# Zydak/Vulkan-Path-Tracer

Measured on AMD Instinct MI355X. Metric: Msamples/s at 1920x1080, higher is better.
Workload: dtype f32; 1 GPU; cornell_1080p_d8; scene=CornellBox (12 triangles, emissive quad 50), black env, width=1920, height=1080, max_depth=8, samples_per_frame=1, batches_per_gpu=14 x 904 frames, partition=rows y % N == rank, one ncclGather at the end, base_seed=1

## Files before the change

### include/vpt_lab.h

```cpp
#ifndef VPT_LAB_H
#define VPT_LAB_H
#include "vpt.h"
#ifdef __cplusplus
extern "C" {
#endif

#define VPT_TRACE_BASE 0u
#define VPT_TRACE_VOTE 1u
#define VPT_TRACE_VOTE8 2u
#define VPT_TRACE_POOL 3u
#define VPT_TRACE_PAIR 4u
#define VPT_TRACE_VOTE4S 5u
int vpt_lab_set_rays(vpt_ctx* ctx, const vpt_ray* rays_host, uint32_t n);
#define VPT_LAB_LANES 1u
#define VPT_LAB_LANE_GRID 2u
#define VPT_LAB_TAIL_GRID 3u
#define VPT_LAB_WHOLE_FRAMES 4u
#define VPT_LAB_WHOLE_SCHED 5u
#define VPT_LAB_WHOLE_PARTS 6u
#define VPT_LAB_WHOLE_CULL 7u
int vpt_lab_set(vpt_ctx* ctx, uint32_t key, uint32_t value);
int vpt_lab_whole_culled(const vpt_ctx* ctx, uint64_t* out);
int vpt_lab_trace(vpt_ctx* ctx, uint32_t variant, uint32_t any_hit, const uint32_t* order_host, uint32_t param, uint32_t reps,
                  vpt_hit* hits_host, float* best_ms, uint64_t* visits);
int vpt_lab_set_holes(vpt_ctx* ctx, const unsigned char* hole_host);
int vpt_lab_trace_shadow(vpt_ctx* ctx, uint32_t light, uint32_t ray_queries, const uint32_t* expect_host, const unsigned char* media_host,
                         const unsigned char* hole_host, unsigned char* vis_host, uint64_t* visits);

#ifdef __cplusplus
}
#endif
#endif
```

### vulkan-path-tracer_amd/_abi.py

```python
import ctypes as C

VPT_OK = 0
ERR_NAMES = {
    -1: "VPT_ERR_INVALID_ARGUMENT", -2: "VPT_ERR_NO_DEVICE", -3: "VPT_ERR_OUT_OF_MEMORY", -4: "VPT_ERR_NO_SCENE",
    -5: "VPT_ERR_DEVICE", -6: "VPT_ERR_UNSUPPORTED", -7: "VPT_ERR_LIMIT",
}

FLAG_SKY_MIS = 1 << 0
FLAG_MESH_MIS = 1 << 1
FLAG_LOCAL_HITS = 1 << 8
FLAG_SHOW_ENV_DIRECTLY = 1 << 2
FLAG_GEOMETRY_NORMALS = 1 << 3
FLAG_ENERGY_COMPENSATION = 1 << 4
FLAG_FURNACE = 1 << 5
FLAG_RAY_QUERIES = 1 << 6
FLAG_TONEMAP_LINEAR_BLOOM_TAP = 1 << 7
FLAGS_DEFAULT = (FLAG_SKY_MIS | FLAG_MESH_MIS | FLAG_SHOW_ENV_DIRECTLY | FLAG_ENERGY_COMPENSATION |
                 FLAG_RAY_QUERIES | FLAG_TONEMAP_LINEAR_BLOOM_TAP)

KERNEL_NAMES = ["primary", "extend", "shade", "connect", "bounce", "resolve", "bloom", "tonemap", "shadow", "join"]
KERNEL_COUNT = 10
PIPELINE_AUTO, PIPELINE_FUSED, PIPELINE_STAGED = 0, 1, 2
PIPELINE_STAGED_R1, PIPELINE_STAGED_SORTED, PIPELINE_WHOLE = 3, 4, 5
LAB_LANES, LAB_LANE_GRID, LAB_TAIL_GRID, LAB_WHOLE_FRAMES, LAB_WHOLE_SCHED, LAB_WHOLE_PARTS, LAB_WHOLE_CULL = 1, 2, 3, 4, 5, 6, 7
ASYNC_MAX_BOUNCES = 32


class Material(C.Structure):
    _fields_ = [
        ("base_color", C.c_float * 3), ("emissive_color", C.c_float * 3), ("specular_color", C.c_float * 3),
        ("medium_color", C.c_float * 3), ("medium_emissive_color", C.c_float * 3),
        ("metallic", C.c_float), ("roughness", C.c_float), ("ior", C.c_float), ("transmission", C.c_float),
        ("anisotropy", C.c_float), ("anisotropy_rotation", C.c_float), ("medium_density", C.c_float),
        ("medium_anisotropy", C.c_float),
        ("base_color_texture", C.c_uint32), ("normal_texture", C.c_uint32), ("roughness_texture", C.c_uint32),
        ("metallic_texture", C.c_uint32), ("emissive_texture", C.c_uint32),
    ]


assert C.sizeof(Material) == 112


class Volume(C.Structure):
    _fields_ = [
        ("corner_min", C.c_float * 3), ("corner_max", C.c_float * 3), ("color", C.c_float * 3), ("emissive_color", C.c_float * 3),
        ("density", C.c_float), ("anisotropy", C.c_float), ("alpha", C.c_float), ("droplet_size", C.c_float),
        ("density_data_index", C.c_int32), ("approximated_scattering", C.c_int32), ("approximated_scattering_falloff", C.c_float),
        ("grid_sharpness", C.c_float), ("has_temperature_data", C.c_int32), ("use_blackbody", C.c_int32), ("temperature_color", C.c_float * 3),
        ("temperature_gamma", C.c_float), ("temperature_scale", C.c_float), ("emissive_color_gamma", C.c_float),
        ("kelvin_min", C.c_int32), ("kelvin_max", C.c_int32),
    ]


assert C.sizeof(Volume) == 120


class Atmosphere(C.Structure):
    _fields_ = [
        ("planet_position", C.c_float * 3), ("planet_radius", C.c_float), ("atmosphere_height", C.c_float),
        ("rayleigh_density_falloff", C.c_float), ("mie_density_falloff", C.c_float), ("ozone_density_falloff", C.c_float),
        ("ozone_peak", C.c_float),
        ("rayleigh_multiplier", C.c_float * 3), ("mie_multiplier", C.c_float * 3), ("ozone_multiplier", C.c_float * 3),
        ("sun_color", C.c_float * 3),
    ]


assert C.sizeof(Atmosphere) == 84


def atmosphere(**kw):
    a = Atmosphere()
    d = dict(planet_position=(0.0, 6360e3 + 1000.0, 0.0), planet_radius=6360e3, atmosphere_height=100e3, rayleigh_density_falloff=8000.0,
             mie_density_falloff=1200.0, ozone_density_falloff=5000.0, ozone_peak=22000.0, rayleigh_multiplier=(1, 1, 1), mie_multiplier=(1, 1, 1),
             ozone_multiplier=(1, 1, 1), sun_color=(1.0, 0.956, 0.88))
    d.update(kw)
    for k, v in d.items():
        if isinstance(v, (tuple, list)):
            getattr(a, k)[:] = v
        else:
            setattr(a, k, v)
    return a
PHASE_HENYEY_GREENSTEIN, PHASE_DRAINE, PHASE_HENYEY_GREENSTEIN_PLUS_DRAINE = 0, 1, 2


def volume(corner_min=(-1, -1, -1), corner_max=(1, 1, 1), color=(0.8, 0.8, 0.8), emissive_color=(0, 0, 0), density=1.0, anisotropy=0.0,
           alpha=1.0, droplet_size=20.0, approximated_scattering=0, approximated_scattering_falloff=0.8, density_data_index=-1, grid_sharpness=1.0,
           has_temperature_data=0, use_blackbody=1, temperature_color=(1.0, 0.5, 0.0), temperature_gamma=1.0, temperature_scale=1.0,
           emissive_color_gamma=1.0, kelvin_min=500, kelvin_max=8000):
    v = Volume()
    v.corner_min[:] = corner_min; v.corner_max[:] = corner_max; v.color[:] = color; v.emissive_color[:] = emissive_color
    v.density, v.anisotropy, v.alpha, v.droplet_size = density, anisotropy, alpha, droplet_size
    v.density_data_index = density_data_index
    v.grid_sharpness = grid_sharpness
    v.has_temperature_data, v.use_blackbody = has_temperature_data, use_blackbody
    v.temperature_color[:] = temperature_color
    v.temperature_gamma, v.temperature_scale, v.emissive_color_gamma = temperature_gamma, temperature_scale, emissive_color_gamma
    v.kelvin_min, v.kelvin_max = kelvin_min, kelvin_max
    v.approximated_scattering, v.approximated_scattering_falloff = approximated_scattering, approximated_scattering_falloff
    return v


class Mesh(C.Structure):
    _fields_ = [("vertices", C.c_void_p), ("vertex_count", C.c_uint32), ("indices", C.c_void_p),
                ("index_count", C.c_uint32)]


class Instance(C.Structure):
    _fields_ = [("mesh_index", C.c_uint32), ("material_index", C.c_uint32), ("transform", C.c_float * 16)]


class Texture(C.Structure):
    _fields_ = [("width", C.c_uint32), ("height", C.c_uint32), ("channels", C.c_uint32), ("data", C.c_void_p)]


class SceneDesc(C.Structure):
    _fields_ = [
        ("meshes", C.POINTER(Mesh)), ("mesh_count", C.c_uint32),
        ("materials", C.POINTER(Material)), ("material_count", C.c_uint32),
        ("instances", C.POINTER(Instance)), ("instance_count", C.c_uint32),
        ("textures", C.POINTER(Texture)), ("texture_count", C.c_uint32),
        ("env_rgba", C.c_void_p), ("env_width", C.c_uint32), ("env_height", C.c_uint32),
        ("lut_reflection", C.c_void_p), ("lut_refraction_outside", C.c_void_p), ("lut_refraction_inside", C.c_void_p),
    ]


class Params(C.Structure):
    _fields_ = [
        ("samples_per_frame", C.c_uint32), ("max_samples", C.c_uint32), ("max_depth", C.c_uint32),
        ("max_luminance", C.c_float), ("focus_distance", C.c_float), ("dof_strength", C.c_float),
        ("sky_azimuth", C.c_float), ("sky_altitude", C.c_float), ("sky_intensity", C.c_float),
        ("screen_chunk_count", C.c_uint32), ("emissive_pdf_bias", C.c_float), ("flags", C.c_uint32),
        ("base_seed", C.c_uint32),
    ]


def default_params(**kw):
    p = Params(1, 5000, 200, 500.0, 1.0, 0.0, 0.0, 0.0, 1.0, 1, 0.0, FLAGS_DEFAULT, 1)
    for k, v in kw.items():
        if not hasattr(p, k):
            raise AttributeError(k)
        setattr(p, k, v)
    return p


class PostParams(C.Structure):
    _fields_ = [("exposure", C.c_float), ("gamma", C.c_float), ("bloom_threshold", C.c_float),
                ("bloom_strength", C.c_float), ("mip_count", C.c_uint32), ("falloff_range", C.c_float), ("schedule", C.c_uint32)]


def default_post_params(**kw):
    p = PostParams(1.0, 2.2, 2.0, 1.0, 10, 5.0, 0)
    for k, v in kw.items():
        if not hasattr(p, k):
            raise AttributeError(k)
        setattr(p, k, v)
    return p


class Config(C.Structure):
    _fields_ = [("device", C.c_int), ("width", C.c_uint32), ("height", C.c_uint32), ("shard_rank", C.c_uint32),
                ("shard_count", C.c_uint32), ("frames_in_flight", C.c_uint32), ("profile", C.c_uint32),
                ("count_traversal", C.c_uint32), ("pipeline", C.c_uint32), ("build_flags", C.c_uint32), ("resident_frames", C.c_uint32)]


class Stats(C.Structure):
    _fields_ = [
        ("samples", C.c_uint64), ("frames", C.c_uint64), ("dispatches", C.c_uint64), ("closest_rays", C.c_uint64),
        ("shadow_rays", C.c_uint64), ("connect_paths", C.c_uint64), ("primary_hits", C.c_uint64), ("primary_survivors", C.c_uint64), ("primary_shadow_rays", C.c_uint64), ("nodes_visited", C.c_uint64), ("tris_tested", C.c_uint64),
        ("shadow_nodes_visited", C.c_uint64), ("shadow_tris_tested", C.c_uint64),
        ("kernel_launches", C.c_uint64 * KERNEL_COUNT), ("kernel_ms", C.c_double * KERNEL_COUNT),
        ("total_vertex_count", C.c_uint64), ("total_index_count", C.c_uint64),
        ("bvh_nodes", C.c_uint32), ("bvh_triangles", C.c_uint32), ("bvh_node_bytes", C.c_uint32),
        ("bvh_tri_bytes", C.c_uint32), ("emissive_mesh_count", C.c_uint32), ("emissive_triangle_count", C.c_uint32),
        ("frames_in_flight", C.c_uint32), ("shard_pixels", C.c_uint32), ("bvh8_nodes", C.c_uint32), ("build_flags", C.c_uint32),
        ("frames_allocated", C.c_uint32), ("resident_frames", C.c_uint32), ("reserved0", C.c_uint32), ("graph_launches", C.c_uint32), ("stack_spills", C.c_uint64 * 2),
        ("set_scene_ms", C.c_double), ("bvh_build_ms", C.c_double),
        ("finish_paths", C.c_uint64), ("finish_closest_rays", C.c_uint64), ("finish_shadow_rays", C.c_uint64),
        ("set_environment_ms", C.c_double),
    ]


class CommInfo(C.Structure):
    _fields_ = [("rccl_version_runtime", C.c_int32), ("rccl_version_compiled", C.c_int32), ("nranks", C.c_int32), ("rank", C.c_int32),
                ("device", C.c_int32), ("reserved", C.c_int32), ("library_path", C.c_char * 232)]


class Ray(C.Structure):
    _fields_ = [("origin", C.c_float * 3), ("tmin", C.c_float), ("direction", C.c_float * 3), ("tmax", C.c_float)]


class Hit(C.Structure):
    _fields_ = [("t", C.c_float), ("u", C.c_float), ("v", C.c_float), ("primitive", C.c_uint32),
                ("instance", C.c_uint32)]


class DensityGridInfo(C.Structure):
    _fields_ = [("dim", C.c_uint32 * 3), ("brick_count", C.c_uint32), ("device_bytes", C.c_uint64), ("max_density", C.c_float), ("reserved", C.c_uint32)]


FEATURES_CENTER, FEATURES_SAMPLE = 0, 1


class FeatureBuffers(C.Structure):
    _fields_ = [("depth", C.c_void_p), ("ids", C.c_void_p), ("normal", C.c_void_p), ("albedo", C.c_void_p), ("device", C.c_uint32), ("reserved", C.c_uint32)]


class PickResult(C.Structure):
    _fields_ = [("instance", C.c_uint32), ("primitive", C.c_uint32), ("material", C.c_uint32), ("mesh", C.c_uint32),
                ("t", C.c_float), ("u", C.c_float), ("v", C.c_float), ("position", C.c_float * 3)]


DENOISE_DEMODULATE, DENOISE_MAX_ITERATIONS = 1, 6
POST_SOURCE_RADIANCE, POST_SOURCE_DENOISED = 0, 1


class DenoiseParams(C.Structure):
    _fields_ = [("iterations", C.c_uint32), ("sigma_color", C.c_float), ("sigma_normal", C.c_float), ("sigma_depth", C.c_float),
                ("flags", C.c_uint32), ("reserved", C.c_uint32)]


def default_denoise_params(**kw):
    p = DenoiseParams(5, 1.0, 0.1, 0.05, DENOISE_DEMODULATE, 0)
    for k, v in kw.items():
        if not hasattr(p, k):
            raise AttributeError(k)
        setattr(p, k, v)
    return p


TEMPORAL_DEMODULATE, TEMPORAL_MATCH_INSTANCE = 1, 2
DENOISE_SOURCE_RADIANCE, DENOISE_SOURCE_TEMPORAL = 0, 1


class TemporalParams(C.Structure):
    _fields_ = [("max_history", C.c_uint32), ("depth_tolerance", C.c_float), ("normal_threshold", C.c_float), ("flags", C.c_uint32), ("reserved", C.c_uint32 * 2)]


def default_temporal_params(**kw):
    p = TemporalParams(32, 0.02, 0.9, TEMPORAL_DEMODULATE | TEMPORAL_MATCH_INSTANCE)
    for k, v in kw.items():
        if not hasattr(p, k):
            raise AttributeError(k)
        setattr(p, k, v)
    return p


class SvgfOptions(C.Structure):
    _fields_ = [("variance", C.c_uint32), ("sigma_luminance", C.c_float), ("min_history", C.c_uint32), ("reserved", C.c_uint32)]


def default_svgf_options(**kw):
    p = SvgfOptions(0, 4.0, 4, 0)
    for k, v in kw.items():
        if not hasattr(p, k):
            raise AttributeError(k)
        setattr(p, k, v)
    return p


class TemporalOptions(C.Structure):
    _fields_ = [("instance_motion", C.c_uint32), ("reserved", C.c_uint32 * 3)]


def default_temporal_options(**kw):
    p = TemporalOptions(0)
    for k, v in kw.items():
        if not hasattr(p, k):
            raise AttributeError(k)
        setattr(p, k, v)
    return p


PROTOTYPES = {
    "vpt_create": (C.c_void_p, [C.POINTER(Config), C.POINTER(C.c_int)]),
    "vpt_destroy": (None, [C.c_void_p]),
    "vpt_last_error": (C.c_char_p, [C.c_void_p]),
    "vpt_set_scene": (C.c_int, [C.c_void_p, C.POINTER(SceneDesc)]),
    "vpt_set_material": (C.c_int, [C.c_void_p, C.c_uint32, C.POINTER(Material)]),
    "vpt_get_material": (C.c_int, [C.c_void_p, C.c_uint32, C.POINTER(Material)]),
    "vpt_set_environment": (C.c_int, [C.c_void_p, C.c_void_p, C.c_uint32, C.c_uint32]),
    "vpt_set_instance_transforms": (C.c_int, [C.c_void_p, C.c_uint32, C.c_uint32, C.c_void_p]),
    "vpt_get_set_transforms_ms": (C.c_int, [C.c_void_p, C.POINTER(C.c_double)]),
    "vpt_set_camera": (C.c_int, [C.c_void_p, C.POINTER(C.c_float), C.POINTER(C.c_float)]),
    "vpt_get_whole_cull": (C.c_int, [C.c_void_p, C.POINTER(C.c_uint32)]),
    "vpt_default_atmosphere": (None, [C.POINTER(Atmosphere)]),
    "vpt_set_atmosphere": (C.c_int, [C.c_void_p, C.c_void_p]),
    "vpt_add_density_grid": (C.c_int, [C.c_void_p, C.c_uint32, C.c_uint32, C.c_uint32, C.c_void_p]),
    "vpt_add_density_bricks": (C.c_int, [C.c_void_p, C.c_uint32, C.c_uint32, C.c_uint32, C.c_uint32, C.c_void_p, C.c_void_p]),
    "vpt_clear_density_grids": (C.c_int, [C.c_void_p]),
    "vpt_get_density_grid_info": (C.c_int, [C.c_void_p, C.c_uint32, C.POINTER(DensityGridInfo)]),
    "vpt_read_density_grid": (C.c_int, [C.c_void_p, C.c_uint32, C.c_void_p, C.c_uint32, C.c_void_p]),
    "vpt_set_volumes": (C.c_int, [C.c_void_p, C.c_void_p, C.c_uint32]),
    "vpt_set_phase_function": (C.c_int, [C.c_void_p, C.c_uint32]),
    "vpt_set_params": (C.c_int, [C.c_void_p, C.POINTER(Params)]),
    "vpt_default_params": (None, [C.POINTER(Params)]),
    "vpt_default_post_params": (None, [C.POINTER(PostParams)]),
    "vpt_resize": (C.c_int, [C.c_void_p, C.c_uint32, C.c_uint32]),
    "vpt_reset": (C.c_int, [C.c_void_p]),
    "vpt_render": (C.c_int, [C.c_void_p, C.c_uint32, C.POINTER(C.c_int)]),
    "vpt_render_async": (C.c_int, [C.c_void_p, C.c_uint32, C.POINTER(C.c_int), C.POINTER(C.c_uint64)]),
    "vpt_postprocess_device": (C.c_int, [C.c_void_p, C.POINTER(PostParams), C.c_void_p, C.POINTER(C.c_uint64)]),
    "vpt_wait": (C.c_int, [C.c_void_p, C.c_uint64]),
    "vpt_output_device": (C.c_void_p, [C.c_void_p]),
    "vpt_get_output": (C.c_int, [C.c_void_p, C.c_void_p]),
    "vpt_get_radiance": (C.c_int, [C.c_void_p, C.c_void_p]),
    "vpt_get_radiance_device": (C.c_int, [C.c_void_p, C.c_void_p]),
    "vpt_set_radiance": (C.c_int, [C.c_void_p, C.c_void_p, C.c_uint32]),
    "vpt_shard_floats": (C.c_size_t, [C.c_void_p]),
    "vpt_get_shard_device": (C.c_int, [C.c_void_p, C.c_void_p]),
    "vpt_assemble_shards": (C.c_int, [C.c_void_p, C.c_void_p, C.c_uint32]),
    "vpt_comm_unique_id": (C.c_int, [C.c_void_p]),
    "vpt_comm_init": (C.c_int, [C.c_void_p, C.c_void_p, C.c_int, C.c_int]),
    "vpt_comm_gather_shards": (C.c_int, [C.c_void_p, C.c_int]),
    "vpt_comm_get_info": (C.c_int, [C.c_void_p, C.POINTER(CommInfo)]),
    "vpt_device_identity": (C.c_int, [C.c_void_p, C.c_char_p, C.c_uint32]),
    "vpt_comm_destroy": (C.c_int, [C.c_void_p]),
    "vpt_multi_gather_shards": (C.c_int, [C.POINTER(C.c_void_p), C.c_uint32, C.c_uint32]),
    "vpt_postprocess": (C.c_int, [C.c_void_p, C.POINTER(PostParams), C.c_void_p, C.c_void_p]),
    "vpt_get_stats": (C.c_int, [C.c_void_p, C.POINTER(Stats)]),
    "vpt_reset_stats": (C.c_int, [C.c_void_p]),
    "vpt_trace_rays": (C.c_int, [C.c_void_p, C.c_void_p, C.c_uint32, C.c_void_p]),
    "vpt_render_features": (C.c_int, [C.c_void_p, C.c_uint32, C.c_uint32, C.POINTER(FeatureBuffers)]),
    "vpt_pick": (C.c_int, [C.c_void_p, C.c_uint32, C.c_uint32, C.POINTER(PickResult)]),
    "vpt_default_denoise_params": (None, [C.POINTER(DenoiseParams)]),
    "vpt_denoise": (C.c_int, [C.c_void_p, C.POINTER(DenoiseParams), C.c_void_p]),
    "vpt_denoise_device": (C.c_int, [C.c_void_p, C.POINTER(DenoiseParams), C.c_void_p, C.POINTER(C.c_uint64)]),
    "vpt_set_post_source": (C.c_int, [C.c_void_p, C.c_uint32]),
    "vpt_default_temporal_params": (None, [C.POINTER(TemporalParams)]),
    "vpt_temporal_accumulate": (C.c_int, [C.c_void_p, C.POINTER(TemporalParams), C.c_void_p]),
    "vpt_temporal_accumulate_device": (C.c_int, [C.c_void_p, C.POINTER(TemporalParams), C.c_void_p, C.POINTER(C.c_uint64)]),
    "vpt_temporal_reset": (C.c_int, [C.c_void_p]),
    "vpt_get_temporal_history": (C.c_int, [C.c_void_p, C.c_void_p]),
    "vpt_set_denoise_source": (C.c_int, [C.c_void_p, C.c_uint32]),
    "vpt_set_base_seed": (C.c_int, [C.c_void_p, C.c_uint32]),
    "vpt_default_svgf_options": (None, [C.POINTER(SvgfOptions)]),
    "vpt_set_svgf_options": (C.c_int, [C.c_void_p, C.POINTER(SvgfOptions)]),
    "vpt_get_svgf_options": (C.c_int, [C.c_void_p, C.POINTER(SvgfOptions)]),
    "vpt_get_temporal_variance": (C.c_int, [C.c_void_p, C.c_void_p]),
    "vpt_get_temporal_moments": (C.c_int, [C.c_void_p, C.c_void_p]),
    "vpt_default_temporal_options": (None, [C.POINTER(TemporalOptions)]),
    "vpt_set_temporal_options": (C.c_int, [C.c_void_p, C.POINTER(TemporalOptions)]),
    "vpt_get_temporal_options": (C.c_int, [C.c_void_p, C.POINTER(TemporalOptions)]),
    "vpt_get_temporal_motion": (C.c_int, [C.c_void_p, C.c_void_p]),
    "vpt_lab_set": (C.c_int, [C.c_void_p, C.c_uint32, C.c_uint32]),
    "vpt_lab_set_rays": (C.c_int, [C.c_void_p, C.c_void_p, C.c_uint32]),
    "vpt_lab_whole_culled": (C.c_int, [C.c_void_p, C.POINTER(C.c_uint64)]),
    "vpt_lab_trace": (C.c_int, [C.c_void_p, C.c_uint32, C.c_uint32, C.c_void_p, C.c_uint32, C.c_uint32, C.c_void_p, C.POINTER(C.c_float), C.POINTER(C.c_uint64)]),
    "vpt_lab_set_holes": (C.c_int, [C.c_void_p, C.c_void_p]),
    "vpt_lab_trace_shadow": (C.c_int, [C.c_void_p, C.c_uint32, C.c_uint32, C.c_void_p, C.c_void_p, C.c_void_p, C.c_void_p, C.POINTER(C.c_uint64)]),
    "vpt_lut_calculate": (C.c_int, [C.c_int] + [C.c_uint32] * 6 + [C.c_void_p]),
}


COMM_ID_BYTES = 128


LAB_ENTRY_POINTS = ("vpt_lab_set", "vpt_lab_set_holes", "vpt_lab_set_rays", "vpt_lab_trace", "vpt_lab_trace_shadow", "vpt_lab_whole_culled")


def bind(lib):
    lib.has_lab = True
    for name, (res, args) in PROTOTYPES.items():
        if name in LAB_ENTRY_POINTS and not hasattr(lib, name):
            lib.has_lab = False
            continue
        fn = getattr(lib, name)
        fn.restype = res
        fn.argtypes = args
    return lib
```

### vulkan-path-tracer_amd/_build.py

```python
import os
import subprocess
import sys

HERE = os.path.dirname(os.path.abspath(__file__))
CSRC = os.path.join(HERE, "csrc")
LIB = os.path.join(HERE, "libvpt_hip.so")
LIB_LAB = os.path.join(HERE, "libvpt_hip_lab.so")
SOURCES = ["kernels_whole.hip", "kernels_finish.hip", "kernels_bounce.hip", "kernels_aux.hip", "kernels_trace.hip", "kernels_stream.hip", "kernels_media.hip", "kernels_post.hip",
           "api_context.hip", "api_scene.hip", "api_render.hip", "api_post.hip", "api_comm.hip", "bvh_build.cpp"]
LAB_SOURCES = ["kernels_lab_r1.hip", "api_lab.hip"]
HEADERS = ["kernels_lut.hip", "device_types.hpp", "path_plan.hpp", "scene_prep.hpp", "grid_prep.hpp", "denoise.hpp", "temporal.hpp", "kernels.hpp", "api_ctx.hpp", "shading.hpp", "traverse.hpp", "bvh_build.hpp", "bvh_refit.hpp", "volume.hpp", "atmosphere.hpp", "wave.hpp", "shade_core.hpp", "vote.hpp", "slab.hpp", "whole_refill.hpp", "whole_args.hpp", "whole_deal.hpp", "camera.hpp", "camera_cull.hpp",
           os.path.join("..", "..", "include", "vpt.h"), os.path.join("..", "..", "include", "vpt_lab.h"), os.path.join("..", "..", "include", "vpt_fp32.h")]
FLAGS = ["--offload-arch=gfx950", "-O3", "-std=c++17", "-fPIC", "-ffp-contract=off", "-fno-fast-math",
         "-fhip-fp32-correctly-rounded-divide-sqrt", "-Wno-unused-result", "-Wno-pass-failed"]
EXTRA_FLAGS = {f: ["-fno-slp-vectorize"] for f in ("kernels_trace.hip", "kernels_stream.hip", "kernels_media.hip", "kernels_whole.hip", "kernels_finish.hip", "kernels_bounce.hip", "kernels_aux.hip", "kernels_lab_r1.hip")}
EXTRA_FLAGS.update({f: ["-Os"] for f in ("api_context.hip", "api_scene.hip", "api_render.hip", "api_post.hip", "api_comm.hip")})
EXTRA_FLAGS["bvh_build.cpp"] = ["-O2"]
EXTRA_FLAGS["kernels_post.hip"] = ["-Xarch_host", "-Os"]


def hipcc():
    for c in (os.environ.get("HIPCC"), "/opt/rocm/bin/hipcc", "hipcc"):
        if c and (os.path.isabs(c) and os.path.exists(c) or not os.path.isabs(c)):
            return c
    raise RuntimeError("hipcc not found")


def _sources(lab):
    return SOURCES + (LAB_SOURCES if lab else [])


def source_id(defines=("-DVPT_LAB=0",)):
    import hashlib
    h = hashlib.sha256()
    for f in sorted(_sources("-DVPT_LAB=1" in defines)) + sorted(HEADERS):
        h.update(open(os.path.join(CSRC, f), "rb").read())
    h.update(repr((FLAGS, sorted(EXTRA_FLAGS.items()), sorted(defines))).encode())
    return h.hexdigest()[:16]


def needs_build(lab=False):
    lib = LIB_LAB if lab else LIB
    if not os.path.exists(lib):
        return True
    t = os.path.getmtime(lib)
    return os.path.getmtime(__file__) > t or any(os.path.getmtime(os.path.join(CSRC, f)) > t for f in _sources(lab) + HEADERS)


def build(force=False, verbose=False, lab=False):
    lib = LIB_LAB if lab else LIB
    if not force and not needs_build(lab):
        return lib
    import fcntl
    os.makedirs(os.path.join(HERE, "build"), exist_ok=True)
    with open(os.path.join(HERE, "build", ".lock"), "w") as lock:
        fcntl.flock(lock, fcntl.LOCK_EX)
        if not force and not needs_build(lab):
            return lib
        return _build_locked(lib, force, verbose, lab)


def _build_locked(lib, force, verbose, lab):
    objs = []
    procs = []
    objdir = os.path.join(HERE, "build", "lab" if lab else "product")
    os.makedirs(objdir, exist_ok=True)
    newest_header = max([os.path.getmtime(__file__)] + [os.path.getmtime(os.path.join(CSRC, h)) for h in HEADERS])
    for src in _sources(lab):
        obj = os.path.join(objdir, src + ".o")
        objs.append(obj)
        if not force and os.path.exists(obj) and os.path.getmtime(obj) > max(newest_header, os.path.getmtime(os.path.join(CSRC, src))):
            continue
        cmd = [hipcc()] + FLAGS + ["-DVPT_LAB=%d" % (1 if lab else 0)] + EXTRA_FLAGS.get(src, []) + (["-x", "hip"] if src.endswith(".cpp") else []) + ["-c", os.path.join(CSRC, src), "-o", obj]
        if verbose:
            print(" ".join(cmd))
        procs.append((src, subprocess.Popen(cmd, stdout=subprocess.PIPE, stderr=subprocess.STDOUT)))
    for src, p in procs:
        out = p.communicate()[0].decode()
        if p.returncode != 0:
            raise RuntimeError("hipcc failed on %s:\n%s" % (src, out))
        if verbose and out.strip():
            print(out)
    return link(lib, objs)


def link(lib, objs):
    exports = os.path.join(HERE, "build", "exports.map")
    with open(exports, "w") as f:
        f.write("{ global: vpt_*; local: *; };\n")
    subprocess.check_call([hipcc(), "--offload-arch=gfx950", "-shared", "-fPIC", "-o", lib] + objs +
                          ["-L/opt/rocm/lib", "-lrccl", "-Wl,-rpath,/opt/rocm/lib", "-Wl,--strip-all", "-Wl,--gc-sections", "-Wl,--version-script=" + exports])
    return lib


if __name__ == "__main__":
    print(build(force="--force" in sys.argv, verbose=True, lab="--lab" in sys.argv))
```

### vulkan-path-tracer_amd/csrc/api_ctx.hpp

```cpp
#pragma once
#include <algorithm>
#include <cstddef>
#include <cstdio>
#include <cstring>
#include <string>
#include <vector>

#include "camera_cull.hpp"
#include "kernels.hpp"
#include "path_plan.hpp"
#include "scene_prep.hpp"

using namespace vpt;

struct ncclComm;

struct BatchState {
    uint32_t frames = 0, dispatch_base = 0, n_slots = 0;
    uint32_t n_first = 0;
    plan::Schedule sd;
    int primary_grid = 0;
    int tail_grid = 0;
    bool count = false;
    bool finished = false;
    uint32_t parity = 0, k3 = 0;
    bool join_pending = false;
    uint64_t iter = 0, iter_cap = 0, min_bounces = 0;
};
struct Grids { int primary, tail; };
struct HostCounters {
    Counters ctr;
    uint32_t alive[2], queue_len[2];
    uint32_t refill_next;
};
constexpr int kTickets = 16;
constexpr int kLanes = 3;

struct Lane {
    hipStream_t stream = nullptr;
    hipStream_t stream2 = nullptr;
    hipEvent_t ev_shade = nullptr, ev_join = nullptr;
    hipEvent_t ev_resolved = nullptr;
    Counters* ctr = nullptr;
    StreamCounters* sctr = nullptr;
    HostCounters* h_ctr = nullptr;
    uint32_t* d_dispatch_base = nullptr;
    uint32_t* spill = nullptr;
    uint32_t* spill2 = nullptr;
    uint32_t stack_overflow_words = 0;

    uint32_t frames_alloc = 0;
    uint32_t resident_alloc = 0;
    bool ps_has_sidx = false, ps_has_media = false;
    uint32_t stream_slack = 0;
    void* ps_block = nullptr;
    PathState ps{};
    uint32_t* queue[2] = {nullptr, nullptr};
    void* ss_block = nullptr;
    StreamState ss{};
    void* ps_legacy = nullptr;
    uint32_t* cqueue = nullptr;
    uint32_t* class_queue[kShadeClasses] = {nullptr, nullptr, nullptr, nullptr, nullptr};
    unsigned char* cls_q = nullptr;
    void* media_block = nullptr;
    MediaState ms{};
    uint32_t media_frames = 0;

    hipGraphExec_t graph = nullptr;
    uint64_t graph_gen = 0;
    uint32_t graph_frames = 0, graph_bounces = 0;
    uint64_t graph_kernel_launches[VPT_KERNEL_COUNT] = {};
    bool graph_broken = false;
    BatchState graph_batch;
    BatchState last_fixed;
    bool last_fixed_valid = false;
};

struct vpt_ctx {
    vpt_config cfg{};
    std::string err;
    int cu_count = 256;

    bool has_scene = false;
    bool buffers_ok = false;
    uint32_t texture_count = 0;
    ncclComm* comm = nullptr;
    int comm_rank = -1, comm_world = 0;
    float* gather_buf = nullptr;
    float4 *lab_ro = nullptr, *lab_rd = nullptr, *lab_hit = nullptr;
    uint32_t *lab_hinst = nullptr, *lab_order = nullptr;
    uint32_t lab_n = 0; float lab_tmin = 0.0f, lab_tmax = 0.0f;
#if VPT_LAB
    std::vector<unsigned char> lab_holes;
#endif
    std::vector<vpt_material> materials;
    std::vector<MeshDesc> meshes;
    std::vector<InstanceDesc> instances;
    scene::EmissiveList emissive;
    uint64_t total_vertices = 0, total_indices = 0;
    uint32_t bvh_depth = 0;
    uint32_t total_tris = 0;
    std::vector<uint32_t> refit_level_off;
    const uint32_t* refit_order = nullptr;
    bool lab_trees_stale = false;

    DeviceScene dsc{};
    std::vector<void*> scene_allocs;
    struct Writable {
        vpt_material* materials = nullptr;
        EmissiveDesc* emissive = nullptr;
        MatResolved* mat_resolved = nullptr;
        EmissiveTri* emissive_tri = nullptr;
        uint32_t* emissive_tri_offset = nullptr;
        float4* tri_ng = nullptr;
        float4* tri_shade = nullptr;
        unsigned char* inst_class = nullptr;
    } dw;
    std::vector<BvhTri> bvh_input;
    bool lds_scene = false;
    bool scene_plain = false;
    std::vector<unsigned char> tex_1x1;
    bool sbvh = false;
    int trav_blocks = 1024;

    vpt_params params{};
    RenderParams P{};
    uint32_t frames_in_flight = 1;
    uint32_t frames_cap = 0;
    uint32_t long_factor = 4;
    int whole_blocks = 0;
    uint32_t lab_whole_sched = 4u;
    uint32_t lab_whole_frames = 0xffffffffu;
    uint32_t lab_whole_parts = 0;
    cull::WorldBox whole_box{};
    bool lab_whole_cull = true;
    bool depth_bounded = true;
    hipEvent_t tick_ev[kTickets] = {};
    uint64_t tick_issued = 0;
    bool async_dirty = false;
    bool out_active = false;
    BatchState out_batch;
    uint64_t out_ticket = 0;
    uint64_t state_gen = 1;
    uint32_t graph_streak = 0;
    uint64_t graph_streak_gen = 0;
    Lane main;
    Lane* extra[kLanes - 1] = {};
    Lane* lane(int k) { return k == 0 ? &main : extra[k - 1]; }
    Lane* order_lane = nullptr;
    hipEvent_t ev_post = nullptr;
    bool post_pending = false;
    uint32_t lane_rr = 0;
    uint32_t lab_lanes = 3, lab_lane_grid = 1, lab_tail_grid = 3;
    unsigned long long* d_spill_count = nullptr;
    bool spill_dirty = true;
    uint64_t spill_cached[2] = {0, 0};
    double set_scene_ms = 0.0, bvh_build_ms = 0.0, set_environment_ms = 0.0, set_transforms_ms = 0.0;

    int shade_media_blocks = 768, media_tail_blocks = 768;
    uint32_t class_present = 0x1fu;
    int shade_stream_blocks = 768, shadow_blocks = 2048, finish_blocks = 768;
    std::vector<vpt_volume> volumes;
    vpt_volume* d_volumes = nullptr;
    std::vector<DensityGrid> grids;
    DensityGrid* d_grids = nullptr;
    uint32_t phase = VPT_PHASE_HENYEY_GREENSTEIN;
    uint32_t* d_launch_off = nullptr;
    int shade_blocks = 1024, primary_blocks = 768, max_blocks = 1536, join_blocks = 2048;
    int primary_blocks_general = 768, primary_blocks_plain = 768;
    int vote_blocks = 2048;
    uint32_t vote_param = 256u + 16u;
    float* image = nullptr;
    float* full_image = nullptr;
    bool full_valid = false;

    uint64_t dispatch_count = 0;
    uint32_t frame_count = 0, samples_accum = 0;
    vpt_stats stats{};

    std::vector<float*> mips;
    std::vector<std::pair<uint32_t, uint32_t>> mip_sizes;
    uint8_t* post_out = nullptr;
    uint32_t post_w = 0, post_h = 0;
    float* dn_block = nullptr;
    float *dn_guide = nullptr, *dn_albedo = nullptr, *dn_depth = nullptr, *dn_ping = nullptr, *dn_pong = nullptr, *dn_out = nullptr;
    uint32_t dn_w = 0, dn_h = 0;
    bool dn_valid = false;
    uint32_t post_source = VPT_POST_SOURCE_RADIANCE;
    float* tp_block = nullptr;
    float *tp_out = nullptr, *tp_hist[2] = {nullptr, nullptr}, *tp_guide[2] = {nullptr, nullptr}, *tp_albedo = nullptr, *tp_depth = nullptr;
    uint32_t *tp_ids = nullptr, *tp_inst[2] = {nullptr, nullptr};
    uint32_t tp_w = 0, tp_h = 0;
    uint32_t tp_latest = 0;
    bool tp_valid = false;
    bool tp_history = false;
    temporal::PrevCamera tp_camera{};
    uint32_t denoise_source = VPT_DENOISE_SOURCE_RADIANCE;
    vpt_svgf_options svgf{0u, 4.0f, 4u, 0u};
    float* sv_block = nullptr;
    float *sv_moments[2] = {nullptr, nullptr}, *sv_variance = nullptr;
    bool sv_valid = false;
    vpt_temporal_options tp_options{0u, {0u, 0u, 0u}};
    temporal::MotionSnapshot tp_snapshot;
    float* tp_motion = nullptr;
    temporal::InstanceMotion* tp_motion_table[2] = {nullptr, nullptr};
    std::vector<temporal::InstanceMotion> tp_motion_host[2];
    size_t tp_motion_cap = 0;
    uint32_t tp_motion_latest = 0;
    bool tp_motion_valid = false;

    std::vector<hipEvent_t> ev_pool;
    struct Pending { int kernel; hipEvent_t a, b; };
    std::vector<Pending> pending;
    size_t ev_next = 0;
};
namespace vpt {
namespace api {

int hip_failed(vpt_ctx* c, hipError_t e, const char* call, const char* file, int line);
#define HIPCHK(ctx, call)                                                                            \
    do {                                                                                             \
        hipError_t e_ = (call);                                                                      \
        if (e_ != hipSuccess) return ::vpt::api::hip_failed((ctx), e_, #call, __FILE__, __LINE__);   \
    } while (0)
int fail(vpt_ctx* c, int code, const char* msg);

inline uint32_t shard_rows_of(uint32_t height, uint32_t rank, uint32_t count) { return rank < height ? (height - rank + count - 1) / count : 0; }
inline const float* whole_image(vpt_ctx* c) { return c->P.shard_count > 1 ? c->full_image : c->image; }

plan::Facts facts_of(const vpt_ctx* c);
hipError_t memset_now(hipStream_t s, void* p, int v, size_t n);
void free_spill(Lane& L);
void free_lab(vpt_ctx* c);
void destroy_graph(Lane& L);
int check_stream_slack(vpt_ctx* c);
plan::Policy policy_of(const vpt_ctx* c);
plan::State plan_state(const vpt_ctx* c);
uint32_t batch_cap(const vpt_ctx* c);
bool path_buffers_hold(const vpt_ctx* c, uint32_t frames);
int ensure_path_buffers(vpt_ctx* c, uint32_t want);
int ensure_media_buffers(vpt_ctx* c, Lane& L);
int ensure_sorted_buffers(vpt_ctx* c, Lane& L);
int ensure_legacy_buffers(vpt_ctx* c, Lane& L);
void reset_accum(vpt_ctx* c, bool keep_history = false);
void free_denoise_buffers(vpt_ctx* c);
void free_temporal_buffers(vpt_ctx* c);
int alloc_spill(vpt_ctx* c, Lane& L, int regions);
Lane* get_lane(vpt_ctx* c, int k);
int ensure_lane_buffers(vpt_ctx* c, Lane& L);
void destroy_lanes(vpt_ctx* c);
void begin_timing(vpt_ctx* c, hipStream_t s, int kernel, hipEvent_t* a, hipEvent_t* b);
void end_timing(hipStream_t s, hipEvent_t b);
void collect_timing(vpt_ctx* c);
#define TIMED(ctx, s, kid, launch_expr)                     \
    do {                                                    \
        hipEvent_t ea_, eb_;                                \
        ::vpt::api::begin_timing(ctx, s, kid, &ea_, &eb_);  \
        launch_expr;                                        \
        ::vpt::api::end_timing(s, eb_);                     \
    } while (0)

void free_scene(vpt_ctx* c);
int refresh_material_tables(vpt_ctx* c);
void enqueue_first_hit(vpt_ctx* c, const FirstHitArgs& a);
int upload_bytes(vpt_ctx* c, const void* src, size_t bytes, size_t total_bytes, void** out);
template <class T>
int upload(vpt_ctx* c, const T* src, size_t n, const T** out, size_t min_elems = 1, T** writable = nullptr) {
    void* d = nullptr;
    int rc = upload_bytes(c, src, n * sizeof(T), std::max(n, min_elems) * sizeof(T), &d);
    if (d) { *out = (T*)d; if (writable) *writable = (T*)d; }
    return rc;
}
template <class T>
int upload(vpt_ctx* c, const std::vector<T>& v, const T** out, size_t min_elems = 1, T** writable = nullptr) {
    return upload(c, v.data(), v.size(), out, min_elems, writable);
}

DeviceScene lane_scene(const vpt_ctx* c, const Lane& L);
cull::Rect whole_cull_rect(const vpt_ctx* c);
uint64_t issue_ticket(vpt_ctx* c, hipStream_t on);
int finish_outstanding(vpt_ctx* c);
int drain(vpt_ctx* c);
int quiesce(vpt_ctx* c);

}
}
```

### vulkan-path-tracer_amd/csrc/api_lab.hip

```cpp
#include "api_ctx.hpp"
#include "bvh_build.hpp"

using namespace vpt::api;

extern "C" {

int vpt_lab_set(vpt_ctx* c, uint32_t key, uint32_t value) {
    if (!c || (value > 3u && key != VPT_LAB_WHOLE_FRAMES && key != VPT_LAB_WHOLE_SCHED && key != VPT_LAB_WHOLE_PARTS)) return VPT_ERR_INVALID_ARGUMENT;
    { int rd = quiesce(c); if (rd) return rd; }
    if (key == VPT_LAB_LANES && value >= 1u) c->lab_lanes = value;
    else if (key == VPT_LAB_LANE_GRID && value >= 1u) c->lab_lane_grid = value;
    else if (key == VPT_LAB_TAIL_GRID && value >= 1u) c->lab_tail_grid = value;
    else if (key == VPT_LAB_WHOLE_SCHED && (value & 15u) >= 1u && (value >> 4) <= 3u) c->lab_whole_sched = value;
    else if (key == VPT_LAB_WHOLE_FRAMES) c->lab_whole_frames = value == 0xffffu ? 0xffffffffu : value;
    else if (key == VPT_LAB_WHOLE_PARTS && value <= plan::kMaxParts) c->lab_whole_parts = value;
    else if (key == VPT_LAB_WHOLE_CULL && value <= 1u) c->lab_whole_cull = value != 0u;
    else return VPT_ERR_INVALID_ARGUMENT;
    c->state_gen++;
    return VPT_OK;
}
int vpt_lab_whole_culled(const vpt_ctx* c, uint64_t* out) {
    if (!c || !out) return VPT_ERR_INVALID_ARGUMENT;
    *out = c->main.h_ctr ? c->main.h_ctr->ctr.whole_culled : 0u;
    return VPT_OK;
}
static constexpr uint32_t kLabGuard = 1024u;
static constexpr uint32_t kLabHole = 0xffffffffu, kLabRayHole = 0xfffffffeu;
static int guard_untouched(vpt_ctx* c, const void* dev, size_t bytes) {
    std::vector<unsigned char> g(bytes);
    HIPCHK(c, hipMemcpy(g.data(), dev, bytes, hipMemcpyDeviceToHost));
    for (unsigned char b : g) if (b != 0xAA) return fail(c, VPT_ERR_DEVICE, "the launch wrote results beyond the last ray of the set");
    return VPT_OK;
}
int vpt_lab_set_rays(vpt_ctx* c, const vpt_ray* rays, uint32_t n) {
    if (!c || !rays || n == 0 || n > 0xffffffffu - kLabGuard) return VPT_ERR_INVALID_ARGUMENT;
    HIPCHK(c, hipSetDevice(c->cfg.device));
    free_lab(c);
    const size_t m = (size_t)n + kLabGuard;
    std::vector<float4> ro(m, make_float4(0.0f, 0.0f, 0.0f, 0.0f)), rd(m, make_float4(0.0f, 0.0f, 0.0f, 0.0f));
    for (uint32_t i = 0; i < n; i++) {
        ro[i] = make_float4(rays[i].origin[0], rays[i].origin[1], rays[i].origin[2], 0.0f);
        rd[i] = make_float4(rays[i].direction[0], rays[i].direction[1], rays[i].direction[2], 0.0f);
    }
    HIPCHK(c, hipMalloc((void**)&c->lab_ro, m * 16)); HIPCHK(c, hipMalloc((void**)&c->lab_rd, m * 16));
    HIPCHK(c, hipMalloc((void**)&c->lab_hit, m * 16)); HIPCHK(c, hipMalloc((void**)&c->lab_hinst, m * 4));
    HIPCHK(c, hipMalloc((void**)&c->lab_order, m * 8));
    c->lab_holes.clear();
    HIPCHK(c, hipMemcpy(c->lab_ro, ro.data(), m * 16, hipMemcpyHostToDevice));
    HIPCHK(c, hipMemcpy(c->lab_rd, rd.data(), m * 16, hipMemcpyHostToDevice));
    c->lab_n = n; c->lab_tmin = rays[0].tmin; c->lab_tmax = rays[0].tmax;
    return VPT_OK;
}
int vpt_lab_set_holes(vpt_ctx* c, const unsigned char* hole) {
    if (!c) return VPT_ERR_INVALID_ARGUMENT;
    if (c->lab_n == 0) return fail(c, VPT_ERR_INVALID_ARGUMENT, "vpt_lab_set_holes before vpt_lab_set_rays");
    { int rd = quiesce(c); if (rd) return rd; }
    HIPCHK(c, hipSetDevice(c->cfg.device));
    c->lab_holes.clear();
    if (!hole) return VPT_OK;
    const uint32_t n = c->lab_n;
    const size_t m = (size_t)n + kLabGuard;
    std::vector<uint32_t> valid(m);
    for (size_t i = 0; i < m; i++) valid[i] = (i < n && hole[i]) ? kLabHole : (uint32_t)i;
    HIPCHK(c, hipMemcpy(c->lab_order + m, valid.data(), m * 4, hipMemcpyHostToDevice));
    c->lab_holes.assign(hole, hole + n);
    return VPT_OK;
}
int vpt_lab_trace(vpt_ctx* c, uint32_t variant, uint32_t any_hit, const uint32_t* order, uint32_t param, uint32_t reps, vpt_hit* hits, float* best_ms,
                  uint64_t* visits) {
    if (!c || variant > VPT_TRACE_VOTE4S || reps == 0) return VPT_ERR_INVALID_ARGUMENT;
    if ((variant == VPT_TRACE_POOL || variant == VPT_TRACE_PAIR) && any_hit) return fail(c, VPT_ERR_UNSUPPORTED, "VPT_TRACE_POOL / _PAIR are closest-hit variants");
    if (!c->has_scene) return fail(c, VPT_ERR_NO_SCENE, "no scene");
    if (c->lds_scene) return fail(c, VPT_ERR_UNSUPPORTED, "the trace lab runs on scenes whose BVH lives in memory");
    if (c->lab_n == 0) return fail(c, VPT_ERR_INVALID_ARGUMENT, "vpt_lab_trace before vpt_lab_set_rays");
    { int rd = quiesce(c); if (rd) return rd; }
    if ((variant == VPT_TRACE_VOTE4S || variant == VPT_TRACE_VOTE8) && c->lab_trees_stale) return fail(c, VPT_ERR_UNSUPPORTED, "instances have moved since vpt_set_scene: this variant's tree is gone until the next one");
    if (variant == VPT_TRACE_VOTE4S && !c->dsc.nodes4s) {
        std::vector<BvhNode> n4, n4s; std::vector<BvhNodeWide> w4; std::vector<BvhTri> lt; int d = 0;
        BvhBuildOptions opt; opt.spatial_splits = c->sbvh; opt.nodes4s = &n4s;
        build_bvh_ex(c->bvh_input, n4, w4, lt, &d, opt);
        int rc4 = upload(c, n4s, &c->dsc.nodes4s);
        if (rc4) return rc4;
    }
    if (variant == VPT_TRACE_VOTE8 && !c->dsc.nodes8) {
        std::vector<BvhNode> n4; std::vector<BvhNodeWide> w4; std::vector<BvhTri> lt; std::vector<BvhNode8> n8; int d = 0;
        build_bvh(c->bvh_input, n4, w4, lt, &d, &n8, c->sbvh);
        if (n8.empty()) return fail(c, VPT_ERR_UNSUPPORTED, "no eight-wide tree for an empty scene");
        int rc8 = upload(c, n8, &c->dsc.nodes8);
        if (rc8) return rc8;
        c->stats.bvh8_nodes = (uint32_t)n8.size();
    }
    const uint32_t n = c->lab_n;
    const bool holes = !c->lab_holes.empty();
    if (holes && variant != VPT_TRACE_VOTE) return fail(c, VPT_ERR_UNSUPPORTED, "only VPT_TRACE_VOTE knows holes: vpt_lab_set_holes(ctx, NULL) first");
    c->spill_dirty = true;
    const size_t m = (size_t)n + kLabGuard;
    if (order) {
        std::vector<uint32_t> o(m);
        for (size_t i = 0; i < m; i++) o[i] = i < n ? order[i] : (uint32_t)i;
        if (holes) for (uint32_t i = 0; i < n; i++) {
            if (o[i] >= n) return fail(c, VPT_ERR_INVALID_ARGUMENT, "order_host is no permutation of the resident rays");
            if (c->lab_holes[o[i]]) o[i] = kLabHole;
        }
        HIPCHK(c, hipMemcpy(c->lab_order, o.data(), m * 4, hipMemcpyHostToDevice));
    }
    TraceArgs a{};
    a.ro = c->lab_ro; a.rd = c->lab_rd; a.order = order ? c->lab_order : nullptr; a.hit = c->lab_hit; a.hinst = c->lab_hinst;
    a.valid = holes && !order ? c->lab_order + m : nullptr;
    a.n = n; a.head = &c->main.ctr->extend_head; a.tmin = c->lab_tmin; a.tmax = c->lab_tmax; a.normalize_dir = 0u; a.param = (variant == VPT_TRACE_POOL || variant == VPT_TRACE_PAIR) ? param : param & 0xfff1ffffu;
    a.cull = variant == VPT_TRACE_VOTE ? (param >> 17) & 1u : 0u;
    a.one_tri = variant == VPT_TRACE_VOTE ? (param >> 19) & 1u : 0u;
    a.packed = variant == VPT_TRACE_VOTE ? (param >> 18) & 1u : 0u;
    const uint32_t blocks = (uint32_t)std::min(trace_blocks_per_cu(variant, any_hit != 0) * c->cu_count, (variant == VPT_TRACE_POOL || variant == VPT_TRACE_PAIR) ? c->max_blocks / 2 : c->max_blocks);
    hipEvent_t e0, e1;
    HIPCHK(c, hipEventCreate(&e0)); HIPCHK(c, hipEventCreate(&e1));
    float best = 1e30f;
    for (uint32_t r = 0; r < reps + (visits ? 1u : 0u); r++) {
        const bool count = visits && r == reps;
        HIPCHK(c, hipMemsetAsync(c->main.ctr, 0, sizeof(Counters), c->main.stream));
        HIPCHK(c, hipMemsetAsync(c->lab_hit + (holes ? 0u : n), 0xAA, (holes ? m : kLabGuard) * 16, c->main.stream));
        HIPCHK(c, hipMemsetAsync(c->lab_hinst + (holes ? 0u : n), 0xAA, (holes ? m : kLabGuard) * 4, c->main.stream));
        HIPCHK(c, hipEventRecord(e0, c->main.stream));
        launch_trace(c->main.stream, blocks, variant, any_hit != 0, count, lane_scene(c, c->main), a, c->main.ctr);
        HIPCHK(c, hipEventRecord(e1, c->main.stream));
        HIPCHK(c, hipStreamSynchronize(c->main.stream));
        HIPCHK(c, hipGetLastError());
        int rg = guard_untouched(c, c->lab_hit + n, kLabGuard * 16);
        if (!rg) rg = guard_untouched(c, c->lab_hinst + n, kLabGuard * 4);
        if (rg) { (void)hipEventDestroy(e0); (void)hipEventDestroy(e1); return rg; }
        float ms = 0.0f;
        HIPCHK(c, hipEventElapsedTime(&ms, e0, e1));
        if (!count) best = std::min(best, ms);
        else {
            Counters h{};
            HIPCHK(c, hipMemcpy(&h, c->main.ctr, sizeof(Counters), hipMemcpyDeviceToHost));
            visits[0] = h.stat_nodes; visits[1] = h.stat_tris;
        }
    }
    (void)hipEventDestroy(e0); (void)hipEventDestroy(e1);
    HIPCHK(c, memset_now(c->main.stream, c->main.ctr, 0, sizeof(Counters)));
    if (best_ms) *best_ms = best;
    if (hits) {
        std::vector<float4> h4(n); std::vector<uint32_t> hi(n, 0xffffffffu);
        HIPCHK(c, hipMemcpy(h4.data(), c->lab_hit, (size_t)n * 16, hipMemcpyDeviceToHost));
        if (!any_hit) HIPCHK(c, hipMemcpy(hi.data(), c->lab_hinst, (size_t)n * 4, hipMemcpyDeviceToHost));
        for (uint32_t i = 0; i < n; i++) {
            hits[i].t = h4[i].x; hits[i].u = h4[i].y; hits[i].v = h4[i].z;
            uint32_t prim; memcpy(&prim, &h4[i].w, 4);
            hits[i].primitive = any_hit ? 0xffffffffu : prim; hits[i].instance = hi[i];
        }
    }
    return VPT_OK;
}

namespace {
struct ShadowLabBuffers {
    float4 *ro = nullptr, *rd = nullptr;
    unsigned char* vis = nullptr;
    StreamCounters* sctr = nullptr;
    ~ShadowLabBuffers() { for (void* p : {(void*)ro, (void*)rd, (void*)vis, (void*)sctr}) if (p) (void)hipFree(p); }
};
}
int vpt_lab_trace_shadow(vpt_ctx* c, uint32_t light, uint32_t ray_queries, const uint32_t* expect, const unsigned char* media, const unsigned char* hole,
                         unsigned char* vis, uint64_t* visits) {
    if (!c || !vis || (light && !expect)) return VPT_ERR_INVALID_ARGUMENT;
    if (!c->has_scene) return fail(c, VPT_ERR_NO_SCENE, "no scene");
    if (c->lds_scene) return fail(c, VPT_ERR_UNSUPPORTED, "the trace lab runs on scenes whose BVH lives in memory");
    if (c->lab_n == 0) return fail(c, VPT_ERR_INVALID_ARGUMENT, "vpt_lab_trace_shadow before vpt_lab_set_rays");
    if (light && !ray_queries) return fail(c, VPT_ERR_UNSUPPORTED, "without ray queries the pipeline queues no light rays");
    const uint32_t n = c->lab_n;
    if (light) for (uint32_t i = 0; i < n; i++)
        if (expect[i] >= c->total_tris) return fail(c, VPT_ERR_INVALID_ARGUMENT, "expect_host: no such triangle");
    { int rd = quiesce(c); if (rd) return rd; }
    HIPCHK(c, hipSetDevice(c->cfg.device));
    const size_t m = (size_t)n + kLabGuard;
    float guard_id; { const uint32_t id = light ? expect[0] : 0xffffffffu; memcpy(&guard_id, &id, 4); }
    std::vector<float4> o(n), d(n), ro(m, make_float4(0.0f, 0.0f, 0.0f, 0.0f)), rd(m, make_float4(0.0f, 0.0f, guard_id, 0.0f));
    HIPCHK(c, hipMemcpy(o.data(), c->lab_ro, (size_t)n * 16, hipMemcpyDeviceToHost));
    HIPCHK(c, hipMemcpy(d.data(), c->lab_rd, (size_t)n * 16, hipMemcpyDeviceToHost));
    for (uint32_t i = 0; i < n; i++) {
        const uint32_t id = (hole && hole[i]) ? kLabRayHole : light ? expect[i] : 0xffffffffu;
        float idf; memcpy(&idf, &id, 4);
        ro[i] = make_float4(o[i].x, o[i].y, o[i].z, d[i].x);
        rd[i] = make_float4(d[i].y, d[i].z, idf, (media && media[i]) ? 1.0f : 0.0f);
    }
    ShadowLabBuffers b;
    HIPCHK(c, hipMalloc((void**)&b.ro, m * 16)); HIPCHK(c, hipMalloc((void**)&b.rd, m * 16));
    HIPCHK(c, hipMalloc((void**)&b.vis, m)); HIPCHK(c, hipMalloc((void**)&b.sctr, sizeof(StreamCounters)));
    HIPCHK(c, hipMemcpy(b.ro, ro.data(), m * 16, hipMemcpyHostToDevice));
    HIPCHK(c, hipMemcpy(b.rd, rd.data(), m * 16, hipMemcpyHostToDevice));
    StreamCounters* const sc = b.sctr;
    hipStream_t s = c->main.stream;
    HIPCHK(c, hipMemsetAsync(b.vis, 0xAA, m, s));
    HIPCHK(c, hipMemsetAsync(sc, 0, sizeof(StreamCounters), s));
    HIPCHK(c, hipMemcpyAsync(light ? &sc->light_len.v : &sc->sky_len.v, &n, 4, hipMemcpyHostToDevice, s));
    HIPCHK(c, hipMemsetAsync(c->main.ctr, 0, sizeof(Counters), s));
    StreamState ss{};
    ss.SKO = b.ro; ss.SKD = b.rd; ss.LTO = b.ro; ss.LTD = b.rd; ss.vis_sky = b.vis; ss.vis_light = b.vis; ss.cap = n;
    c->spill_dirty = true;
    launch_trace_shadow(s, (uint32_t)c->shadow_blocks, light != 0u, visits != nullptr, lane_scene(c, c->main), ss, c->main.ctr, sc, c->vote_param, ray_queries ? 1u : 0u);
    HIPCHK(c, hipStreamSynchronize(s));
    HIPCHK(c, hipGetLastError());
    if (visits) {
        Counters h{};
        HIPCHK(c, hipMemcpy(&h, c->main.ctr, sizeof(Counters), hipMemcpyDeviceToHost));
        visits[0] = h.stat_shadow_nodes; visits[1] = h.stat_shadow_tris;
    }
    HIPCHK(c, memset_now(s, c->main.ctr, 0, sizeof(Counters)));
    HIPCHK(c, hipMemcpy(vis, b.vis, (size_t)n, hipMemcpyDeviceToHost));
    return guard_untouched(c, b.vis + n, kLabGuard);
}

}
```

### vulkan-path-tracer_amd/csrc/api_render.hip

```cpp
#include "api_ctx.hpp"

using namespace vpt::api;
using plan::Kind;

namespace {


uint32_t split_dispatch_slots(const RenderParams& P, uint32_t dispatch) {
    const uint32_t S = P.split, ch = dispatch % (S * S), cx = ch % S, cy = ch / S;
    const uint32_t lw = cx < P.width ? (P.width - cx + S - 1) / S : 0, lh = cy < P.height ? (P.height - cy + S - 1) / S : 0;
    return lw * lh;
}
uint32_t batch_slots(const RenderParams& P, uint32_t frames, uint32_t dispatch_base) {
    if (P.split <= 1) return frames * P.shard_pixels;
    uint32_t n = 0;
    for (uint32_t k = 0; k < frames; k++) n += split_dispatch_slots(P, dispatch_base + k);
    return n;
}
int decide_batch(vpt_ctx* c, const Lane& L, const plan::Facts& f, uint32_t frames, uint32_t dispatch_base, bool capturing, plan::Schedule& sd) {
    if (frames == 0 || frames > L.frames_alloc) return fail(c, VPT_ERR_DEVICE, "internal: batch larger than the path buffers");
    sd = plan::decide(f, frames, L.frames_alloc, L.resident_alloc, batch_slots(c->P, frames, dispatch_base), &L != &c->main, capturing);
    return sd.err != VPT_OK ? fail(c, sd.err, sd.msg) : VPT_OK;
}
PathState part_state(const vpt_ctx* c, const Lane& L, uint32_t first_frame) {
    PathState ps = L.ps;
    const size_t at = (size_t)first_frame * c->P.shard_pixels;
    ps.ACC += at; ps.M += at; ps.maniso += at;
    return ps;
}
void resolve_part(vpt_ctx* c, Lane& L, const BatchState& b, uint32_t i, hipStream_t on) {
    const uint32_t first = b.sd.parts.first[i];
    const uint32_t* guard = plan::runs_fused(b.sd.kind) ? &L.ctr->alive3[b.k3] : plan::runs_streams(b.sd.kind) ? &L.sctr->alive[b.parity].v : &L.ctr->ray_count[b.parity];
    TIMED(c, on, VPT_K_RESOLVE, launch_resolve(on, c->P, part_state(c, L, first), c->image, b.sd.parts.first[i + 1] - first, b.dispatch_base + first, guard));
}
int batch_begin(vpt_ctx* c, Lane& L, const plan::Schedule& sd, uint32_t frames, uint32_t dispatch_base, Grids grids, BatchState& b) {
    hipStream_t s = L.stream;
    b = BatchState{};
    b.frames = frames; b.dispatch_base = dispatch_base; b.sd = sd;
    b.primary_grid = grids.primary; b.tail_grid = grids.tail;
    c->spill_dirty = true;
    const uint32_t n_slots = batch_slots(c->P, frames, dispatch_base);
    const cull::Rect wrect = sd.kind == Kind::Whole ? whole_cull_rect(c) : cull::everything(c->P.width, c->P.height);
    uint32_t n_split_dealt = 0;
    if (c->P.split > 1) {
        std::vector<uint32_t> off(frames + 1, 0u);
        for (uint32_t k = 0; k < frames; k++)
            off[k + 1] = off[k] + (wrect.all ? split_dispatch_slots(c->P, dispatch_base + k) : deal::split_rect_px(wrect, (dispatch_base + k) % (c->P.split * c->P.split), c->P.split));
        n_split_dealt = off[frames];
        HIPCHK(c, hipMemcpyAsync(c->d_launch_off, off.data(), off.size() * 4, hipMemcpyHostToDevice, s));
        HIPCHK(c, hipStreamSynchronize(s));
    }
    b.n_slots = n_slots;
    b.n_first = sd.regen ? sd.resident * c->P.shard_pixels : n_slots;
    b.count = c->cfg.count_traversal != 0;
    if (sd.kind == Kind::MediaStreams) {
        int rl = ensure_media_buffers(c, L); if (rl != VPT_OK) return rl;
        if (frames > L.media_frames) return fail(c, VPT_ERR_DEVICE, "internal: media batch larger than the media streams");
    }
    if (sd.kind == Kind::StagedR1) { int rl = ensure_legacy_buffers(c, L); if (rl != VPT_OK) return rl; }
    if (sd.kind == Kind::StreamsSorted) { int rl = ensure_sorted_buffers(c, L); if (rl != VPT_OK) return rl; }
    b.min_bounces = (uint64_t)c->P.max_depth * c->P.samples_per_frame;
    b.iter_cap = (b.min_bounces * 4ull + 1024ull) * ((frames + sd.resident - 1) / sd.resident);
    if (n_slots == 0) return VPT_OK;
    HIPCHK(c, hipMemsetAsync(L.ctr, 0, offsetof(Counters, stat_closest), s));
    const DeviceScene dsc = lane_scene(c, L);
    if (sd.kind == Kind::Whole) {
        b.parity = 1; b.k3 = 1; b.iter = 1;
        const bool dealt = !wrect.all, split = c->P.split > 1;
        const cull::Packed rect = cull::pack(wrect);
        for (uint32_t i = 0; i < sd.parts.n; i++) {
            const uint32_t first = sd.parts.first[i], part_frames = sd.parts.n > 1u ? sd.parts.first[i + 1] - first : frames;
            const uint32_t part_slots = sd.parts.n > 1u ? part_frames * c->P.shard_pixels : n_slots;
            const deal::Deal dl = dealt ? deal::make(wrect, c->P.shard_rank, c->P.shard_count, c->P.width, part_slots) : deal::Deal{};
            const uint32_t n_part = !dealt ? part_slots : split ? n_split_dealt : part_frames * dl.rect_px;
            const uint64_t culled = part_slots - n_part;
            if (dealt && (n_part == 0u || split)) HIPCHK(c, hipMemsetAsync(part_state(c, L, first).ACC, 0, (size_t)(split ? frames * c->P.shard_pixels : part_slots) * 16, s));
            const uint32_t grid = std::max(1u, std::min<uint32_t>((uint32_t)std::min(c->whole_blocks, b.primary_grid), (n_part + 255u) / 256u));
            const uint32_t n_waves = grid * 4u, rounds = ((n_part + 63u) / 64u) / n_waves, mode = c->lab_whole_sched >> 4;
            const uint32_t static_rounds = (mode == 0u || mode == 3u) ? std::min(rounds, 1u) : mode == 1u ? (rounds >= 2u ? rounds - 1u : 0u) : rounds / 2u;
            if (i) HIPCHK(c, hipMemsetAsync(&L.ctr->extend_head, 0, 4, s));
            TIMED(c, s, VPT_K_PRIMARY, launch_whole(s, grid, b.count, dsc, c->P, part_state(c, L, first), L.ctr, n_part, dispatch_base + first, c->scene_plain, static_rounds, std::max(1u, c->lab_whole_sched & 15u) | (mode == 3u ? 0x100u : 0u), rect, dl, culled));
            if (i + 1u < sd.parts.n) {
                HIPCHK(c, hipEventRecord(L.ev_shade, s));
                HIPCHK(c, hipStreamWaitEvent(L.stream2, L.ev_shade, 0));
                resolve_part(c, L, b, i, L.stream2);
            }
        }
    } else if (sd.kind == Kind::Fused) {
        TIMED(c, s, VPT_K_PRIMARY, launch_bounce(s, (uint32_t)b.primary_grid, c->lds_scene, b.count, true, dsc, c->P, L.ps, L.ss, nullptr, L.queue[1], L.ctr, 0u, b.n_first, dispatch_base, 0u, c->scene_plain));
        b.parity = 1; b.k3 = 1; b.iter = 1;
    } else if (plan::runs_streams(sd.kind)) {
        TIMED(c, s, VPT_K_PRIMARY, launch_raygen_stream(s, c->P, L.ps, L.ss, L.queue[0], b.n_first, dispatch_base, sd.kind == Kind::MediaStreams));
        launch_stream_begin(s, L.sctr, b.n_first, n_slots);
        b.parity = 0;
    } else {
#if VPT_LAB
        TIMED(c, s, VPT_K_PRIMARY, launch_raygen(s, c->P, L.ps, L.queue[0], L.ctr, n_slots, dispatch_base));
#endif
        b.parity = 0;
    }
    return VPT_OK;
}

int batch_bounces(vpt_ctx* c, Lane& L, BatchState& b, uint32_t bounces) {
    hipStream_t s = L.stream;
    const Kind kind = b.sd.kind;
    const bool count = b.count, sorted = kind == Kind::StreamsSorted, overlap = b.sd.overlap, stream = plan::runs_streams(kind);
    uint32_t& parity = b.parity;
    const uint32_t n_slots = b.n_first;
    if (n_slots == 0 || kind == Kind::Whole) return VPT_OK;
    const DeviceScene dsc = lane_scene(c, L);
    for (uint32_t j = 0; j < bounces; j++) {
        b.iter++;
        if (kind == Kind::Fused) {
            const int grid = (b.tail_grid > 0 && b.iter >= 3) ? b.tail_grid : b.primary_grid;
            TIMED(c, s, VPT_K_BOUNCE, launch_bounce(s, (uint32_t)grid, c->lds_scene, count, false, dsc, c->P, L.ps, L.ss, L.queue[parity], L.queue[parity ^ 1u], L.ctr, parity, 0u, 0u, b.k3, c->scene_plain));
            parity ^= 1u; b.k3 = (b.k3 + 1u) % 3u;
            continue;
        }
        if (kind == Kind::MediaStreams) {
            launch_prepare_stream(s, L.sctr, parity);
            TraceArgs a{};
            a.ro = L.ss.RA[parity]; a.rd = L.ss.RB[parity]; a.order = nullptr; a.valid = L.queue[parity]; a.hit = L.ss.SH; a.hinst = L.ss.SHI; a.cls = nullptr;
            a.n = 0; a.n_dev = &L.sctr->queue_len[parity].v; a.store_gid = 1u; a.param = c->vote_param;
            a.head = &L.sctr->shade_head.v; a.tmin = 0.00001f; a.tmax = 1000000.0f; a.normalize_dir = 0u;
            if (!(c->P.flags & VPT_FLAG_RAY_QUERIES)) { a.tmax = 1000.0f; a.normalize_dir = 1u; }
            TIMED(c, s, VPT_K_EXTEND, launch_trace(s, (uint32_t)c->vote_blocks, VPT_TRACE_VOTE, false, count, dsc, a, L.ctr));
            TIMED(c, s, VPT_K_SHADE, launch_media_scatter(s, (uint32_t)c->shade_blocks, dsc, L.ps, L.ss, L.ms, L.queue[parity], L.sctr, parity));
            a.head = &L.sctr->extend_head.v; a.tmin = 0.01f; a.tmax = 100000.0f; a.normalize_dir = 1u;
            TIMED(c, s, VPT_K_EXTEND, launch_trace(s, (uint32_t)c->vote_blocks, VPT_TRACE_VOTE, false, count, dsc, a, L.ctr));
            launch_layout_media(s, L.sctr, parity, (uint32_t)c->shade_media_blocks * 4u, (uint32_t)c->media_tail_blocks * 4u);
            TIMED(c, s, VPT_K_SHADE, launch_shade_media(s, (uint32_t)c->shade_media_blocks, dsc, c->P, L.ps, L.ss, L.ms, L.queue[parity], L.ctr, L.sctr, parity));
            TIMED(c, s, VPT_K_SHADOW, launch_trace_shadow(s, (uint32_t)c->shadow_blocks, false, count, dsc, L.ss, L.ctr, L.sctr, c->vote_param, (c->P.flags & VPT_FLAG_RAY_QUERIES) ? 1u : 0u));
            TIMED(c, s, VPT_K_SHADOW, launch_trace_shadow(s, (uint32_t)c->shadow_blocks, true, count, dsc, L.ss, L.ctr, L.sctr, c->vote_param, (c->P.flags & VPT_FLAG_RAY_QUERIES) ? 1u : 0u));
            TIMED(c, s, VPT_K_JOIN, launch_media_tail(s, (uint32_t)c->media_tail_blocks, dsc, c->P, L.ps, L.ss, L.ms, L.queue[parity], L.queue[parity ^ 1u], L.ctr, L.sctr, parity));
            parity ^= 1u;
            continue;
        }
        if (stream && b.finished) continue;
        if (stream && b.sd.finish_at != 0u && b.iter > b.sd.finish_at) {
            if (b.join_pending) { HIPCHK(c, hipStreamWaitEvent(s, L.ev_join, 0)); b.join_pending = false; }
            TIMED(c, s, VPT_K_BOUNCE, launch_finish(s, (uint32_t)c->finish_blocks, count, dsc, c->P, L.ps, L.ss, L.queue[parity], L.sctr, L.ctr, parity));
            b.finished = true;
            continue;
        }
        if (stream) {
            launch_prepare_stream(s, L.sctr, parity);
            TraceArgs a{};
            a.ro = L.ss.RA[parity]; a.rd = L.ss.RB[parity]; a.order = nullptr; a.valid = L.queue[parity]; a.hit = L.ss.SH; a.hinst = L.ss.SHI; a.cls = L.cls_q;
            a.n = 0; a.n_dev = &L.sctr->queue_len[parity].v; a.head = &L.sctr->extend_head.v;
            a.tmin = 0.01f; a.tmax = 100000.0f; a.normalize_dir = 1u; a.store_gid = 1u; a.param = c->vote_param;
            if (!sorted) a.cls = nullptr;
            TIMED(c, s, VPT_K_EXTEND, launch_trace(s, (uint32_t)c->vote_blocks, VPT_TRACE_VOTE, false, count, dsc, a, L.ctr));
            if (overlap && b.join_pending) { HIPCHK(c, hipStreamWaitEvent(s, L.ev_join, 0)); b.join_pending = false; }
            if (sorted) {
                TIMED(c, s, VPT_K_SHADE, launch_classify(s, L.queue[parity], L.cls_q, L.class_queue, L.sctr, parity, n_slots + L.stream_slack, (uint32_t)c->shade_stream_blocks * 4u));
                for (uint32_t k = 0; k < kShadeClasses; k++)
                    if (c->class_present & (1u << k))
                        TIMED(c, s, VPT_K_SHADE, launch_shade_stream(s, (uint32_t)c->shade_stream_blocks, k, true, dsc, c->P, L.ps, L.ss, L.queue[parity], L.class_queue[k], L.queue[parity ^ 1u], L.ctr, L.sctr, parity));
            } else {
                launch_layout_single(s, L.sctr, parity, (uint32_t)c->shade_stream_blocks * 4u);
                TIMED(c, s, VPT_K_SHADE, launch_shade_stream(s, (uint32_t)c->shade_stream_blocks, 0u, false, dsc, c->P, L.ps, L.ss, L.queue[parity], nullptr, L.queue[parity ^ 1u], L.ctr, L.sctr, parity));
            }
            hipStream_t sb = s;
            DeviceScene dsc_shadow = dsc;
            if (overlap) {
                HIPCHK(c, hipEventRecord(L.ev_shade, s));
                HIPCHK(c, hipStreamWaitEvent(L.stream2, L.ev_shade, 0));
                sb = L.stream2;
                dsc_shadow.stack_overflow = L.spill2;
            }
            if (b.sd.regen) TIMED(c, s, VPT_K_PRIMARY, launch_refill(s, 2048u, c->P, L.ps, L.ss, L.queue[parity ^ 1u], L.sctr, parity ^ 1u, b.n_first, b.dispatch_base));
            TIMED(c, s, VPT_K_SHADOW, launch_trace_shadow(sb, (uint32_t)c->shadow_blocks, false, count, dsc_shadow, L.ss, L.ctr, L.sctr, c->vote_param, (c->P.flags & VPT_FLAG_RAY_QUERIES) ? 1u : 0u));
            TIMED(c, s, VPT_K_SHADOW, launch_trace_shadow(sb, (uint32_t)c->shadow_blocks, true, count, dsc_shadow, L.ss, L.ctr, L.sctr, c->vote_param, (c->P.flags & VPT_FLAG_RAY_QUERIES) ? 1u : 0u));
            TIMED(c, s, VPT_K_JOIN, launch_join(sb, (uint32_t)c->join_blocks, c->P, L.ps, L.ss, L.sctr, L.queue[parity], L.queue[parity ^ 1u], parity));
            if (overlap) { HIPCHK(c, hipEventRecord(L.ev_join, L.stream2)); b.join_pending = true; }
            parity ^= 1u;
            continue;
        }
#if VPT_LAB
        launch_prepare(s, L.ctr, parity);
        TIMED(c, s, VPT_K_EXTEND, launch_extend(s, (uint32_t)c->trav_blocks, c->lds_scene, count, dsc, L.ps, L.queue[parity], L.ctr, parity));
        TIMED(c, s, VPT_K_SHADE, launch_shade(s, (uint32_t)c->shade_blocks, dsc, c->P, L.ps, L.queue[parity], L.queue[parity ^ 1u], L.cqueue, L.ctr, parity));
        TIMED(c, s, VPT_K_CONNECT, launch_connect(s, (uint32_t)c->trav_blocks, c->lds_scene, count, dsc, c->P, L.ps, L.cqueue, L.ctr, parity));
#endif
        parity ^= 1u;
    }
    return VPT_OK;
}

int batch_resolve(vpt_ctx* c, Lane& L, BatchState& b) {
    hipStream_t s = L.stream;
    if (b.n_slots == 0) return VPT_OK;
#if VPT_LAB
    if (b.sd.kind == Kind::StagedR1) launch_fold(s, L.ctr);
#endif
    if (b.sd.overlap && b.join_pending) { HIPCHK(c, hipStreamWaitEvent(s, L.ev_join, 0)); b.join_pending = false; }
    const bool stream = plan::runs_streams(b.sd.kind);
    if (b.sd.parts.n > 1u) {
        HIPCHK(c, hipEventRecord(L.ev_join, L.stream2));
        HIPCHK(c, hipStreamWaitEvent(s, L.ev_join, 0));
    }
    resolve_part(c, L, b, b.sd.parts.n - 1u, s);
    HIPCHK(c, hipMemcpyAsync(&L.h_ctr->ctr, L.ctr, sizeof(Counters), hipMemcpyDeviceToHost, s));
    if (stream) {
        HIPCHK(c, hipMemcpyAsync(&L.h_ctr->alive[0], &L.sctr->alive[b.parity].v, 4, hipMemcpyDeviceToHost, s));
        HIPCHK(c, hipMemcpyAsync(&L.h_ctr->queue_len[0], &L.sctr->queue_len[b.parity].v, 4, hipMemcpyDeviceToHost, s));
        HIPCHK(c, hipMemcpyAsync(&L.h_ctr->refill_next, &L.sctr->refill_next, 4, hipMemcpyDeviceToHost, s));
    }
    return VPT_OK;
}

void update_ray_stats(vpt_ctx* c) {
    unsigned long long v[9] = {0, 0, 0, 0, 0, 0, 0, 0, 0};
    for (int k = 0; k < kLanes; k++)
        if (const Lane* L = c->lane(k)) {
            const Counters& h = L->h_ctr->ctr;
            v[0] += h.stat_closest; v[1] += h.stat_shadow; v[2] += h.stat_connect; v[3] += h.stat_primary_hits; v[4] += h.stat_primary_alive; v[5] += h.stat_primary_rays;
            v[6] += h.stat_finish_paths; v[7] += h.stat_finish_closest; v[8] += h.stat_finish_shadow;
        }
    c->stats.closest_rays = v[0]; c->stats.shadow_rays = v[1]; c->stats.connect_paths = v[2];
    c->stats.primary_hits = v[3]; c->stats.primary_survivors = v[4]; c->stats.primary_shadow_rays = v[5];
    c->stats.finish_paths = v[6]; c->stats.finish_closest_rays = v[7]; c->stats.finish_shadow_rays = v[8];
}

int batch_check(vpt_ctx* c, Lane& L, BatchState& b, uint32_t* alive) {
    *alive = 0;
    if (b.n_slots == 0) return VPT_OK;
    HIPCHK(c, hipStreamSynchronize(L.stream));
    collect_timing(c);
    const Counters& h = L.h_ctr->ctr;
    update_ray_stats(c);
    const bool counted = c->cfg.count_traversal != 0;
    c->stats.nodes_visited = counted ? h.stat_nodes : 0;
    c->stats.tris_tested = counted ? h.stat_tris : 0;
    c->stats.shadow_nodes_visited = counted ? h.stat_shadow_nodes : 0;
    c->stats.shadow_tris_tested = counted ? h.stat_shadow_tris : 0;
    uint32_t n = plan::runs_fused(b.sd.kind) ? h.alive3[b.k3] : h.ray_count[b.parity];
    if (plan::runs_streams(b.sd.kind)) {
        n = L.h_ctr->alive[0];
        const uint64_t len = L.h_ctr->queue_len[0];
        const uint64_t room = b.sd.kind == Kind::MediaStreams ? (uint64_t)L.media_frames * c->P.shard_pixels + L.stream_slack : (uint64_t)L.ps.capacity + L.stream_slack;
        if (len > room || len > (uint64_t)L.ps.capacity + L.stream_slack) { (void)hipStreamSynchronize(L.stream2); return fail(c, VPT_ERR_DEVICE, "internal: stream overflow"); }
    }
    if (n > b.n_first) { (void)hipStreamSynchronize(L.stream2); return fail(c, VPT_ERR_DEVICE, "internal: queue overflow"); }
    if (n != 0 && b.iter > b.iter_cap) { (void)hipStreamSynchronize(L.stream2); return fail(c, VPT_ERR_DEVICE, "internal: bounce loop did not terminate"); }
    *alive = n;
    return VPT_OK;
}

int batch_finish(vpt_ctx* c, Lane& L, BatchState& b, bool resolve_enqueued) {
    while (true) {
        if (!resolve_enqueued) { int rc = batch_resolve(c, L, b); if (rc) return rc; }
        resolve_enqueued = false;
        uint32_t n = 0;
        int rc = batch_check(c, L, b, &n);
        if (rc) return rc;
        if (n == 0) break;
        if (b.sd.finisher && (!b.sd.regen || L.h_ctr->refill_next >= b.n_slots) && !b.finished && b.sd.finish_at == 0u && n < plan::kFinishBelowPaths) b.sd.finish_at = (uint32_t)b.iter;
        rc = batch_bounces(c, L, b, b.sd.regen ? 8u : 4u);
        if (rc) return rc;
    }
    HIPCHK(c, hipGetLastError());
    return VPT_OK;
}

int render_batch(vpt_ctx* c, uint32_t frames, uint32_t dispatch_base) {
    Lane& L = c->main;
    plan::Schedule sd;
    int rc = decide_batch(c, L, facts_of(c), frames, dispatch_base, false, sd);
    if (rc) return rc;
    BatchState b;
    rc = batch_begin(c, L, sd, frames, dispatch_base, Grids{c->primary_blocks, 0}, b);
    if (rc) return rc;
    if (b.n_slots == 0) return VPT_OK;
    const uint32_t first = (uint32_t)std::min<uint64_t>(std::max<uint64_t>(b.min_bounces - (plan::runs_fused(sd.kind) ? 1 : 0), 1), 8);
    rc = batch_bounces(c, L, b, first);
    if (rc) return rc;
    rc = batch_finish(c, L, b, false);
    if (rc) return rc;
    c->stats.samples += (uint64_t)b.n_slots * c->P.samples_per_frame;
    return VPT_OK;
}

int enqueue_fixed(vpt_ctx* c, Lane& L, const plan::Schedule& sd, uint32_t frames, uint32_t dispatch_base, uint32_t bounces_total, Grids grids, BatchState& b) {
    int rc = batch_begin(c, L, sd, frames, dispatch_base, grids, b);
    if (rc) return rc;
    if (b.n_slots == 0) return VPT_OK;
    return batch_bounces(c, L, b, plan::runs_fused(sd.kind) ? bounces_total - 1u : bounces_total);
}
int enqueue_graph(vpt_ctx* c, Lane& L, const plan::Facts& f, uint32_t frames, uint32_t dispatch_base, uint32_t bounces_total, Grids grids, bool* used, BatchState& b) {
    *used = false;
    if (L.graph_broken) return VPT_OK;
    if (!L.graph || L.graph_gen != c->state_gen || L.graph_frames != frames || L.graph_bounces != bounces_total) {
        destroy_graph(L);
        uint64_t before[VPT_KERNEL_COUNT];
        memcpy(before, c->stats.kernel_launches, sizeof(before));
        c->P.dispatch_base_dev = L.d_dispatch_base;
        hipGraph_t g = nullptr;
        bool ok = hipStreamBeginCapture(L.stream, hipStreamCaptureModeThreadLocal) == hipSuccess;
        plan::Schedule sd;
        int rc = ok ? decide_batch(c, L, f, frames, 0u, true, sd) : VPT_ERR_DEVICE;
        if (rc == VPT_OK) rc = enqueue_fixed(c, L, sd, frames, 0u, bounces_total, grids, L.graph_batch);
        if (ok && hipStreamEndCapture(L.stream, &g) != hipSuccess) { ok = false; g = nullptr; }
        c->P.dispatch_base_dev = nullptr;
        for (int k = 0; k < VPT_KERNEL_COUNT; k++) { L.graph_kernel_launches[k] = c->stats.kernel_launches[k] - before[k]; c->stats.kernel_launches[k] = before[k]; }
        if (ok && rc == VPT_OK && g && hipGraphInstantiate(&L.graph, g, nullptr, nullptr, 0) != hipSuccess) { ok = false; L.graph = nullptr; }
        if (g) (void)hipGraphDestroy(g);
        if (!ok || rc != VPT_OK || !L.graph) {
            (void)hipGetLastError();
            destroy_graph(L);
            L.graph_broken = true;
            c->err.clear();
            return VPT_OK;
        }
        L.graph_gen = c->state_gen; L.graph_frames = frames; L.graph_bounces = bounces_total;
    }
    HIPCHK(c, hipMemsetD32Async((hipDeviceptr_t)L.d_dispatch_base, (int)dispatch_base, 1, L.stream));
    HIPCHK(c, hipGraphLaunch(L.graph, L.stream));
    for (int k = 0; k < VPT_KERNEL_COUNT; k++) c->stats.kernel_launches[k] += L.graph_kernel_launches[k];
    c->stats.graph_launches++;
    b = L.graph_batch;
    b.dispatch_base = dispatch_base;
    *used = true;
    return VPT_OK;
}

int next_batch(vpt_ctx* c, uint32_t left, uint32_t* nf) {
    *nf = 0;
    if (c->samples_accum >= c->params.max_samples) return VPT_OK;
    const uint64_t S2 = (uint64_t)c->params.screen_chunk_count * c->params.screen_chunk_count;
    const uint64_t frames_needed = ((uint64_t)c->params.max_samples + c->params.samples_per_frame - 1) / c->params.samples_per_frame;
    const uint64_t disp_left = frames_needed * S2 - c->dispatch_count;
    uint32_t n = (uint32_t)std::min<uint64_t>(std::min<uint64_t>(left, batch_cap(c)), disp_left);
    if (!path_buffers_hold(c, n)) {
        int rc = drain(c);
        if (rc) return rc;
        if ((rc = ensure_path_buffers(c, n))) return rc;
    }
    n = plan::fit_batch(policy_of(c), plan_state(c), n);
    if (plan::media_on_streams(facts_of(c))) {
        int rm = ensure_media_buffers(c, c->main);
        if (rm) return rm;
        n = std::min(n, c->main.media_frames);
    }
    *nf = n;
    return VPT_OK;
}
void advance_counts(vpt_ctx* c, uint32_t nf) {
    const uint64_t S2 = (uint64_t)c->params.screen_chunk_count * c->params.screen_chunk_count;
    c->dispatch_count += nf;
    c->frame_count = (uint32_t)(c->dispatch_count / S2);
    c->samples_accum = c->frame_count * c->params.samples_per_frame;
    c->full_valid = false;
}

}

namespace vpt {
namespace api {

DeviceScene lane_scene(const vpt_ctx* c, const Lane& L) {
    DeviceScene d = c->dsc;
    d.stack_overflow = L.spill;
    return d;
}
cull::Rect whole_cull_rect(const vpt_ctx* c) {
    cull::WorldBox box = c->whole_box;
    box.valid = box.valid && c->has_scene && c->lab_whole_cull && c->cfg.count_traversal == 0;
    return cull::screen_bound(c->P.view_inv, c->P.proj_inv, c->P.width, c->P.height, c->P.focus_distance, c->P.dof_strength, c->P.flags, c->dsc.env_black != 0u, box);
}

uint64_t issue_ticket(vpt_ctx* c, hipStream_t on) {
    c->tick_issued++;
    (void)hipEventRecord(c->tick_ev[c->tick_issued % kTickets], on);
    c->async_dirty = true;
    return c->tick_issued;
}
int finish_outstanding(vpt_ctx* c) {
    if (!c->out_active) return VPT_OK;
    c->out_active = false;
    return batch_finish(c, c->main, c->out_batch, true);
}
int drain(vpt_ctx* c) {
    int rc = finish_outstanding(c);
    if (rc) return rc;
    if (!c->async_dirty) return VPT_OK;
    c->async_dirty = false;
    for (int k = 0; k < kLanes; k++) {
        Lane* L = c->lane(k);
        if (!L) continue;
        HIPCHK(c, hipStreamSynchronize(L->stream));
        if (!L->last_fixed_valid) continue;
        L->last_fixed_valid = false;
        const BatchState& f = L->last_fixed;
        if (plan::runs_streams(f.sd.kind)) {
            if (L->h_ctr->alive[0] != 0u) return fail(c, VPT_ERR_DEVICE, "internal: a path outlived a fixed-schedule batch");
            if ((uint64_t)L->h_ctr->queue_len[0] > (uint64_t)L->ps.capacity + L->stream_slack) return fail(c, VPT_ERR_DEVICE, "internal: stream overflow");
        } else if (plan::runs_fused(f.sd.kind) && L->h_ctr->ctr.alive3[f.k3] != 0u) return fail(c, VPT_ERR_DEVICE, "internal: a path outlived a fixed-schedule batch");
    }
    c->order_lane = nullptr; c->post_pending = false;
    HIPCHK(c, hipStreamSynchronize(c->main.stream2));
    collect_timing(c);
    update_ray_stats(c);
    HIPCHK(c, hipGetLastError());
    return VPT_OK;
}
int quiesce(vpt_ctx* c) {
    HIPCHK(c, hipSetDevice(c->cfg.device));
    return drain(c);
}

}
}

extern "C" {

int vpt_render(vpt_ctx* c, uint32_t dispatches, int* done) {
    if (!c) return VPT_ERR_INVALID_ARGUMENT;
    if (!c->has_scene) return fail(c, VPT_ERR_NO_SCENE, "vpt_render before vpt_set_scene");
    if (!c->buffers_ok) return fail(c, VPT_ERR_DEVICE, "no render buffers: the last vpt_resize failed");
    { int rd = quiesce(c); if (rd) return rd; }
    if (done) *done = 0;
    uint32_t left = dispatches;
    while (left > 0) {
        uint32_t nf = 0;
        int rc = next_batch(c, left, &nf);
        if (rc) return rc;
        if (nf == 0) { if (done) *done = 1; break; }
        rc = render_batch(c, nf, (uint32_t)c->dispatch_count);
        if (rc) return rc;
        advance_counts(c, nf);
        left -= nf;
    }
    return VPT_OK;
}

int vpt_render_async(vpt_ctx* c, uint32_t dispatches, int* done, uint64_t* ticket) {
    if (!c) return VPT_ERR_INVALID_ARGUMENT;
    if (!c->has_scene) return fail(c, VPT_ERR_NO_SCENE, "vpt_render_async before vpt_set_scene");
    if (!c->buffers_ok) return fail(c, VPT_ERR_DEVICE, "no render buffers: the last vpt_resize failed");
    HIPCHK(c, hipSetDevice(c->cfg.device));
    if (done) *done = 0;
    uint32_t left = dispatches;
    while (left > 0) {
        int rc = finish_outstanding(c);
        if (rc) return rc;
        uint32_t nf = 0;
        if ((rc = next_batch(c, left, &nf))) return rc;
        if (nf == 0) { if (done) *done = 1; break; }
        const uint32_t base = (uint32_t)c->dispatch_count;
        if (c->graph_streak_gen == c->state_gen) c->graph_streak++; else { c->graph_streak = 0; c->graph_streak_gen = c->state_gen; }
        const plan::Facts f = facts_of(c);
        plan::Schedule sd;
        if ((rc = decide_batch(c, c->main, f, nf, base, false, sd))) return rc;
        const plan::AsyncShape shape = plan::async_shape(f, sd, nf, c->main.resident_alloc, c->graph_streak);
        const bool fixed = shape.fixed;
        const uint32_t enq = shape.bounces_to_enqueue;
        Lane* X = &c->main;
        if (shape.lanes_ok) {
            const int max_lanes = (int)std::max(1u, std::min(c->lab_lanes, (uint32_t)kLanes));
            Lane* idle = nullptr;
            uint32_t have = 0;
            for (int k = 0; k < max_lanes; k++) {
                Lane* L = c->lane(k);
                if (!L) { if (!idle) idle = get_lane(c, k); break; }
                have++;
                if (!idle && hipEventQuery(L->ev_resolved) == hipSuccess) idle = L;
            }
            (void)hipGetLastError();
            if (!idle) idle = c->lane((int)(c->lane_rr++ % have));
            X = idle;
            if (X != &c->main) {
                if ((rc = ensure_lane_buffers(c, *X))) return rc;
                if ((rc = decide_batch(c, *X, f, nf, base, false, sd))) return rc;
            }
        }
        if (X == &c->main && c->order_lane && c->order_lane != X) HIPCHK(c, hipStreamWaitEvent(X->stream, c->order_lane->ev_resolved, 0));
        BatchState b;
        bool graphed = false;
        Grids grids{c->primary_blocks, 0};
        auto part = [&](uint32_t div) { return std::max(c->cu_count, (c->primary_blocks / (int)std::max(1u, div) / std::max(c->cu_count, 1)) * c->cu_count); };
        if (shape.partial_grids) {
            grids.primary = part(std::max(1u, c->lab_lane_grid));
            grids.tail = c->lab_tail_grid > 1u ? std::min(grids.primary, part(c->lab_tail_grid)) : 0;
        }
        if (shape.graph_ok && (rc = enqueue_graph(c, *X, f, nf, base, enq, grids, &graphed, b))) return rc;
        if (!graphed && (rc = enqueue_fixed(c, *X, sd, nf, base, enq, grids, b))) return rc;
        if (fixed && b.n_slots) {
            if (c->order_lane && c->order_lane != X) HIPCHK(c, hipStreamWaitEvent(X->stream, c->order_lane->ev_resolved, 0));
            if (c->post_pending && X != &c->main) HIPCHK(c, hipStreamWaitEvent(X->stream, c->ev_post, 0));
        }
        if ((rc = batch_resolve(c, *X, b))) return rc;
        if (fixed && b.n_slots) {
            HIPCHK(c, hipEventRecord(X->ev_resolved, X->stream));
            c->order_lane = X;
            X->last_fixed = b; X->last_fixed_valid = true;
        }
        c->stats.samples += (uint64_t)b.n_slots * c->P.samples_per_frame;
        advance_counts(c, nf);
        left -= nf;
        const uint64_t t = issue_ticket(c, X->stream);
        if (!fixed && b.n_slots) { c->out_active = true; c->out_batch = b; c->out_ticket = t; }
    }
    if (ticket) *ticket = c->tick_issued;
    return VPT_OK;
}

int vpt_wait(vpt_ctx* c, uint64_t ticket) {
    if (!c) return VPT_ERR_INVALID_ARGUMENT;
    HIPCHK(c, hipSetDevice(c->cfg.device));
    if (ticket == 0 || ticket >= c->tick_issued) return drain(c);
    if (c->out_active && c->out_ticket <= ticket) { int rc = finish_outstanding(c); if (rc) return rc; }
    HIPCHK(c, hipEventSynchronize(c->tick_ev[ticket % kTickets]));
    return VPT_OK;
}

int vpt_get_radiance_device(vpt_ctx* c, void* dst) {
    if (!c || !dst) return VPT_ERR_INVALID_ARGUMENT;
    if (!c->buffers_ok) return fail(c, VPT_ERR_DEVICE, "no render buffers: the last vpt_resize failed");
    if (c->P.shard_count > 1 && !c->full_valid) return fail(c, VPT_ERR_INVALID_ARGUMENT, "sharded context: call vpt_assemble_shards first");
    { int rd = quiesce(c); if (rd) return rd; }
    HIPCHK(c, hipMemcpyAsync(dst, whole_image(c), (size_t)c->P.width * c->P.height * 16, hipMemcpyDeviceToDevice, c->main.stream));
    HIPCHK(c, hipStreamSynchronize(c->main.stream));
    return VPT_OK;
}
int vpt_get_radiance(vpt_ctx* c, float* dst) {
    if (!c || !dst) return VPT_ERR_INVALID_ARGUMENT;
    if (!c->buffers_ok) return fail(c, VPT_ERR_DEVICE, "no render buffers: the last vpt_resize failed");
    if (c->P.shard_count > 1 && !c->full_valid) return fail(c, VPT_ERR_INVALID_ARGUMENT, "sharded context: call vpt_assemble_shards first");
    { int rd = quiesce(c); if (rd) return rd; }
    HIPCHK(c, hipMemcpy(dst, whole_image(c), (size_t)c->P.width * c->P.height * 16, hipMemcpyDeviceToHost));
    return VPT_OK;
}
int vpt_set_radiance(vpt_ctx* c, const float* src, uint32_t frame_count) {
    if (!c || !src) return VPT_ERR_INVALID_ARGUMENT;
    if (!c->buffers_ok) return fail(c, VPT_ERR_DEVICE, "no render buffers: the last vpt_resize failed");
    { int rd = quiesce(c); if (rd) return rd; }
    const uint32_t W = c->P.width;
    if (c->P.shard_count == 1) {
        HIPCHK(c, hipMemcpy(c->image, src, (size_t)W * c->P.height * 16, hipMemcpyHostToDevice));
    } else {
        HIPCHK(c, hipMemcpy(c->full_image, src, (size_t)W * c->P.height * 16, hipMemcpyHostToDevice));
        HIPCHK(c, hipMemcpy2D(c->image, (size_t)W * 16, src + (size_t)c->P.shard_rank * W * 4, (size_t)W * 16 * c->P.shard_count, (size_t)W * 16,
                              c->P.shard_rows, hipMemcpyHostToDevice));
        c->full_valid = true;
    }
    c->frame_count = frame_count;
    c->dispatch_count = (uint64_t)frame_count * c->params.screen_chunk_count * c->params.screen_chunk_count;
    c->samples_accum = frame_count * c->params.samples_per_frame;
    c->tp_history = false;
    return VPT_OK;
}

int vpt_get_stats(vpt_ctx* c, vpt_stats* out) {
    if (!c || !out) return VPT_ERR_INVALID_ARGUMENT;
    if (c->async_dirty || c->out_active) {
        HIPCHK(c, hipSetDevice(c->cfg.device));
        int rd = drain(c); if (rd) return rd;
    }
    vpt_stats s = c->stats;
    s.frames = c->frame_count; s.dispatches = c->dispatch_count;
    s.total_vertex_count = c->total_vertices; s.total_index_count = c->total_indices;
    s.bvh_nodes = c->dsc.node_count; s.bvh_triangles = c->dsc.tri_count;
    s.bvh_node_bytes = c->lds_scene ? sizeof(BvhNodeWide) : sizeof(BvhNode); s.bvh_tri_bytes = sizeof(BvhTri);
    s.emissive_mesh_count = (uint32_t)c->emissive.list.size(); s.emissive_triangle_count = c->emissive.tris;
    s.frames_in_flight = batch_cap(c); s.shard_pixels = c->P.shard_pixels;
    s.build_flags = (c->sbvh ? VPT_BUILD_SBVH : 0u) | (c->cfg.build_flags & (VPT_BUILD_GENERAL_KERNELS | VPT_BUILD_STREAMS_ONLY));
    s.frames_allocated = c->main.frames_alloc; s.resident_frames = c->main.resident_alloc;
    s.set_scene_ms = c->set_scene_ms; s.bvh_build_ms = c->bvh_build_ms; s.set_environment_ms = c->set_environment_ms;
    if (c->has_scene && c->main.spill && c->spill_dirty) {
        HIPCHK(c, hipSetDevice(c->cfg.device));
        unsigned long long h[2] = {0ull, 0ull};
        HIPCHK(c, hipMemsetAsync(c->d_spill_count, 0, 16, c->main.stream));
        for (int k = 0; k < kLanes; k++) {
            const Lane* L = c->lane(k);
            if (!L || !L->spill) continue;
            launch_count_spilled(c->main.stream, L->spill, L->stack_overflow_words, c->d_spill_count);
            if (L->spill2 != L->spill) launch_count_spilled(c->main.stream, L->spill2, L->stack_overflow_words, c->d_spill_count + 1);
        }
        HIPCHK(c, hipMemcpyAsync(h, c->d_spill_count, 16, hipMemcpyDeviceToHost, c->main.stream));
        HIPCHK(c, hipStreamSynchronize(c->main.stream));
        c->spill_cached[0] = h[0]; c->spill_cached[1] = h[1];
        c->spill_dirty = false;
    }
    s.stack_spills[0] = c->has_scene ? c->spill_cached[0] : 0; s.stack_spills[1] = c->has_scene ? c->spill_cached[1] : 0;
    *out = s;
    return VPT_OK;
}
int vpt_get_set_transforms_ms(const vpt_ctx* c, double* out_ms) {
    if (!c || !out_ms) return VPT_ERR_INVALID_ARGUMENT;
    *out_ms = c->set_transforms_ms;
    return VPT_OK;
}
int vpt_reset_stats(vpt_ctx* c) {
    if (!c) return VPT_ERR_INVALID_ARGUMENT;
    { int rd = quiesce(c); if (rd) return rd; }
    c->stats = vpt_stats{};
    for (int k = 0; k < kLanes; k++)
        if (Lane* L = c->lane(k)) { HIPCHK(c, memset_now(L->stream, L->ctr, 0, sizeof(Counters))); memset(L->h_ctr, 0, sizeof(HostCounters)); }
    return VPT_OK;
}

int vpt_get_whole_cull(const vpt_ctx* c, uint32_t* rect) {
    if (!c || !rect) return VPT_ERR_INVALID_ARGUMENT;
    if (!c->has_scene) return VPT_ERR_NO_SCENE;
    const cull::Rect r = whole_cull_rect(c);
    rect[0] = r.x0; rect[1] = r.y0; rect[2] = r.x1; rect[3] = r.y1;
    return VPT_OK;
}

}
```

### vulkan-path-tracer_amd/csrc/kernels.hpp

```cpp
#pragma once
#include "device_types.hpp"
#include "denoise.hpp"
#include "temporal.hpp"
#include "whole_deal.hpp"
#include "../../include/vpt_lab.h"
#ifndef VPT_LAB
#define VPT_LAB 0
#endif

namespace vpt {

void launch_bounce(hipStream_t s, uint32_t blocks, bool lds_scene, bool count, bool first, const DeviceScene& sc, const RenderParams& P,
                   const PathState& ps, const StreamState& ss, const uint32_t* queue, uint32_t* queue_next, Counters* ctr, uint32_t parity, uint32_t n_slots,
                   uint32_t dispatch_base, uint32_t k3, bool plain = false);
int bounce_blocks_per_cu(bool lds_scene, const DeviceScene& sc, bool plain = false);
void launch_whole(hipStream_t s, uint32_t blocks, bool count, const DeviceScene& sc, const RenderParams& P, const PathState& ps, Counters* ctr, uint32_t n_slots,
                  uint32_t dispatch_base, bool plain, uint32_t static_rounds, uint32_t chunk_tiles, cull::Packed rect, const deal::Deal& deal, uint64_t culled);
int whole_blocks_per_cu(const DeviceScene& sc, bool plain);
void launch_finish(hipStream_t s, uint32_t blocks, bool count, const DeviceScene& sc, const RenderParams& P, const PathState& ps, const StreamState& ss, const uint32_t* queue,
                   StreamCounters* sctr, Counters* ctr, uint32_t parity);
int finish_blocks_per_cu(const DeviceScene& sc);
void launch_resolve(hipStream_t s, const RenderParams& P, const PathState& ps, float* image, uint32_t frames, uint32_t frame_base, const uint32_t* guard);
struct FirstHitArgs {
    const vpt_ray* rays; vpt_hit* hits; uint32_t n;
    uint32_t mode, frame;
    float* depth; uint4* ids; float4* normal; float4* albedo;
    float4* pick; uint32_t pixel;
};
void launch_first_hit(hipStream_t s, uint32_t blocks, const DeviceScene& sc, const RenderParams& P, const FirstHitArgs& a);
void launch_trace_rays(hipStream_t s, uint32_t blocks, const DeviceScene& sc, const vpt_ray* rays, uint32_t n, vpt_hit* hits);
void launch_read_density_grid(hipStream_t s, const DensityGrid& g, const int32_t* ijk, uint32_t n, float* out);
void launch_scatter_rows(hipStream_t s, const float* gathered, float* full, uint32_t w, uint32_t h, uint32_t shard_count, uint32_t stride_px);
void launch_precompute_materials(hipStream_t s, const DeviceScene& sc, uint32_t flags, MatResolved* out, uint32_t n);
void launch_precompute_tri_ng(hipStream_t s, const DeviceScene& sc, float4* out);
void launch_precompute_tri_shade(hipStream_t s, const DeviceScene& sc, float4* out);
void launch_precompute_emissive(hipStream_t s, const DeviceScene& sc, EmissiveTri* out, uint32_t total);
void launch_retransform_tris(hipStream_t s, const DeviceScene& sc, uint32_t total_tris, uint32_t n_inst, uint32_t first, uint32_t count, const float* xf, BvhTri* out, uint32_t* words);
void launch_refit_level(hipStream_t s, const DeviceScene& sc, const uint32_t* order, uint32_t begin, uint32_t end, const BvhTri* tris, float pad, float* boxes, BvhNode* nodes_out, BvhNodeWide* wide_out);
size_t traverse_lds_bytes(const DeviceScene& sc, bool lds_scene, int stack_rows);
size_t stack_overflow_bytes(uint32_t blocks);
constexpr int kSpillPatternByte = 0x7f;
constexpr uint32_t kSpillPattern = 0x7f7f7f7f;
void launch_count_spilled(hipStream_t s, const uint32_t* region, uint32_t words, unsigned long long* out);
#if VPT_LAB
void launch_raygen(hipStream_t s, const RenderParams& P, const PathState& ps, uint32_t* queue, Counters* ctr, uint32_t n_slots, uint32_t dispatch_base);
void launch_prepare(hipStream_t s, Counters* ctr, uint32_t parity);
void launch_fold(hipStream_t s, Counters* ctr);
void launch_extend(hipStream_t s, uint32_t blocks, bool lds_scene, bool count, const DeviceScene& sc, const PathState& ps,
                   const uint32_t* queue, Counters* ctr, uint32_t parity);
void launch_shade(hipStream_t s, uint32_t blocks, const DeviceScene& sc, const RenderParams& P, const PathState& ps,
                  const uint32_t* queue, uint32_t* queue_next, uint32_t* cqueue, Counters* ctr, uint32_t parity);
void launch_connect(hipStream_t s, uint32_t blocks, bool lds_scene, bool count, const DeviceScene& sc, const RenderParams& P,
                    const PathState& ps, const uint32_t* cqueue, Counters* ctr, uint32_t parity);
int traverse_blocks_per_cu(bool lds_scene, const DeviceScene& sc);
int shade_blocks_per_cu();
#endif

struct TraceArgs {
    const float4* ro;
    const float4* rd;
    const uint32_t* order;
    const uint32_t* valid;
    float4* hit;
    uint32_t* hinst;
    uint32_t n;
    const uint32_t* n_dev;
    uint32_t* head;
    float tmin, tmax;
    uint32_t normalize_dir;
    uint32_t store_gid;
    uint32_t param;
    unsigned char* cls;
    uint32_t cull;
    uint32_t one_tri;
    uint32_t packed;
};
void launch_trace(hipStream_t s, uint32_t blocks, uint32_t variant, bool any, bool count, const DeviceScene& sc, const TraceArgs& a, Counters* ctr);
int trace_blocks_per_cu(uint32_t variant, bool any);

void launch_stream_begin(hipStream_t s, StreamCounters* sc, uint32_t n_first, uint32_t n_total);
void launch_refill(hipStream_t s, uint32_t blocks, const RenderParams& P, const PathState& ps, const StreamState& ss, uint32_t* queue_next, StreamCounters* sc, uint32_t parity_next,
                   uint32_t cap, uint32_t dispatch_base);
void launch_raygen_stream(hipStream_t s, const RenderParams& P, const PathState& ps, const StreamState& ss, uint32_t* queue, uint32_t n_slots, uint32_t dispatch_base, bool media);
void launch_prepare_stream(hipStream_t s, StreamCounters* sc, uint32_t parity);
void launch_classify(hipStream_t s, const uint32_t* queue, const unsigned char* cls, uint32_t* const* class_queue, StreamCounters* sc, uint32_t parity, uint32_t max_entries, uint32_t shade_waves);
void launch_layout_single(hipStream_t s, StreamCounters* sc, uint32_t parity, uint32_t shade_waves);
void launch_shade_stream(hipStream_t s, uint32_t blocks, uint32_t cls, bool sorted, const DeviceScene& sc, const RenderParams& P, const PathState& ps, const StreamState& ss,
                         const uint32_t* queue, const uint32_t* order, uint32_t* queue_next, Counters* ctr, StreamCounters* sctr, uint32_t parity);
void launch_classify_instances(hipStream_t s, const DeviceScene& sc, unsigned char* out, uint32_t n);
void launch_trace_shadow(hipStream_t s, uint32_t blocks, bool light, bool count, const DeviceScene& sc, const StreamState& ss, Counters* ctr,
                         StreamCounters* sctr, uint32_t param, uint32_t ray_queries = 1u);
void launch_join(hipStream_t s, uint32_t blocks, const RenderParams& P, const PathState& ps, const StreamState& ss, const StreamCounters* sctr, const uint32_t* queue,
                 const uint32_t* queue_next, uint32_t parity);
int shade_stream_blocks_per_cu();
int join_blocks_per_cu();
void launch_media_scatter(hipStream_t s, uint32_t blocks, const DeviceScene& sc, const PathState& ps, const StreamState& ss, const MediaState& ms, const uint32_t* queue,
                          const StreamCounters* sctr, uint32_t parity);
void launch_layout_media(hipStream_t s, StreamCounters* sctr, uint32_t parity, uint32_t shade_waves, uint32_t tail_waves);
void launch_shade_media(hipStream_t s, uint32_t blocks, const DeviceScene& sc, const RenderParams& P, const PathState& ps, const StreamState& ss, const MediaState& ms,
                        const uint32_t* queue, Counters* ctr, StreamCounters* sctr, uint32_t parity);
void launch_media_tail(hipStream_t s, uint32_t blocks, const DeviceScene& sc, const RenderParams& P, const PathState& ps, const StreamState& ss, const MediaState& ms,
                       const uint32_t* queue, uint32_t* queue_next, Counters* ctr, StreamCounters* sctr, uint32_t parity);
int shade_media_blocks_per_cu();
int media_tail_blocks_per_cu();
int trace_shadow_blocks_per_cu();

void launch_lut(hipStream_t s, int kind, float* table, uint32_t sx, uint32_t sy, uint32_t sz, uint32_t sample_count, uint32_t time_hash,
                uint32_t first_dispatch, uint32_t n_dispatches);

void launch_bloom_threshold(hipStream_t s, const float* in, float* out, uint32_t w, uint32_t h, float threshold, float falloff);
void launch_bloom_down(hipStream_t s, const float* in, uint32_t iw, uint32_t ih, float* out, uint32_t ow, uint32_t oh, float strength);
void launch_bloom_up(hipStream_t s, const float* in, uint32_t iw, uint32_t ih, float* out, uint32_t ow, uint32_t oh, float strength);
constexpr uint32_t kBloomChainMax = 4;
constexpr uint32_t kBloomDownChainMax = 3;
constexpr uint32_t kBloomDownChainTexels = 160000;
void launch_bloom_down_chain(hipStream_t s, const float* in, uint32_t iw, uint32_t ih, float* const* outs, const uint32_t* w, const uint32_t* h, uint32_t n, float strength);
void launch_bloom_up_chain(hipStream_t s, float* const* mips, const uint32_t* w, const uint32_t* h, uint32_t n, float strength);
void launch_bloom_down_first(hipStream_t s, const float* hdr, uint32_t iw, uint32_t ih, float* out, uint32_t ow, uint32_t oh, float strength, float threshold, float falloff);
bool bloom_tail_is_staged(uint32_t bw, uint32_t bh);
void launch_bloom_tail(hipStream_t s, float* base, float* top_out, uint32_t bw, uint32_t bh, const uint32_t* w, const uint32_t* h, uint32_t levels, float strength);
void launch_post_final(hipStream_t s, const float* hdr, const float* mip1, uint32_t mw, uint32_t mh, float* bloom0_out, uint8_t* out, uint32_t w, uint32_t h,
                       float threshold, float falloff, float strength, float exposure, float gamma, bool linear_tap);
constexpr uint32_t kBloomTailMaxTexels = 2048, kBloomTailMaxLevels = 8;
void launch_tonemap(hipStream_t s, const float* hdr, const float* bloom0, uint8_t* out, uint32_t w, uint32_t h, float exposure,
                    float gamma, bool linear_tap);
void launch_denoise_prepare(hipStream_t s, const float* c, const float* depth, float* albedo, float* guide, float* e, uint32_t w, uint32_t h, bool demodulate, const float* variance);
void launch_denoise_atrous(hipStream_t s, const float* in, const float* guide, const float* albedo, float* out, uint32_t w, uint32_t h, const denoise::Pass& ps, bool remodulate,
                           bool variance, float sigma_luminance, bool last);
void launch_temporal(hipStream_t s, const float* cur, const float* depth, const float* albedo, const uint32_t* ids, const float* prev_hist, const float* prev_guide, const uint32_t* prev_inst,
                     float* hist, float* guide, uint32_t* inst, float* out, const temporal::Frame& f, const float* prev_moments, float* moments, float* variance, float min_len,
                     const temporal::InstanceMotion* motion_table, uint32_t motion_count, float* motion);

}
```

### vulkan-path-tracer_amd/csrc/kernels_whole.hip

```cpp
#include "kernels.hpp"
#include "traverse.hpp"
#include "wave.hpp"
#include "shade_core.hpp"
#include "whole_refill.hpp"
#include "whole_args.hpp"
#include "camera_cull.hpp"

namespace vpt {

#define VPT_KERNARG __attribute__((address_space(4)))
template <> struct OneSampleFrames<VPT_KERNARG WholeParams> { static constexpr bool value = true; };

template <class Pm, class Ps>
__device__ __forceinline__ V3 whole_finish(const Pm& P, const Ps& ps, uint32_t slot, V3 E, V3 thr_prev, V3 light_prev, const ShadeOut& o) {
    const V3 light = light_prev + path_contribution(E, thr_prev, o.cflags, P.max_luminance);
    if (o.terminated) ps.ACC[slot] = finite3(light) ? f4(v3s(0.0f) + light, 0.0f) : make_float4(0.0f, 0.0f, 0.0f, 0.0f);
    return light;
}
__device__ __attribute__((noinline)) void whole_zero_run(float4* acc, uint32_t first, uint32_t end) {
    for (uint32_t i = first + lane_id(); i < end; i += 64u) acc[i] = make_float4(0.0f, 0.0f, 0.0f, 0.0f);
}

template <bool COUNT, bool STRICT, bool PLAIN>
__global__ __launch_bounds__(kTraverseBlock, 3) void k_whole(WholeLaunch wl) {
    const WholeArgs& a = wl.a;
    const DeviceScene sc = a.sc;
    const RenderParams P = a.P;
    Counters* const ctr = a.ctr;
    extern __shared__ __align__(16) unsigned char smem[];
    const TravStackT<kWholeStackRows> stack = make_stack<kWholeStackRows>(smem, sc.stack_overflow);
    float4* lds_nodes = reinterpret_cast<float4*>(smem + kWholeStackRows * kTraverseBlock * 4);
    float4* lds_tris = lds_nodes + sc.node_count * 8;
    __shared__ CameraBlock cam;
    if (threadIdx.x == 0u) fill_camera_block(cam, P.view_inv, P.proj_inv, P.width, P.height, P.focus_distance, P.dof_strength);
    const VPT_KERNARG WholeArgs* ka = (const VPT_KERNARG WholeArgs*)__builtin_amdgcn_kernarg_segment_ptr();
    stage_scene<true>(sc, lds_nodes, lds_tris);
    constexpr uint32_t kWaves = kTraverseBlock / 64u;
    __shared__ uint32_t r_slot[kWaves][128], r_prim[kWaves][128], r_inst[kWaves][128];
    __shared__ float r_t[kWaves][128], r_u[kWaves][128], r_v[kWaves][128];
    __shared__ float4 r_ra[kWaves][128], r_rb[kWaves][128], r_rt[kWaves][128];
    __shared__ uint32_t f_slot[kWaves][refill::kTile], f_rng[kWaves][refill::kTile];
    __shared__ float f_ox[kWaves][refill::kTile], f_oy[kWaves][refill::kTile], f_oz[kWaves][refill::kTile];
    __shared__ float f_dx[kWaves][refill::kTile], f_dy[kWaves][refill::kTile], f_dz[kWaves][refill::kTile];
    const uint32_t wave = __builtin_amdgcn_readfirstlane(threadIdx.x >> 6);
    const refill::Shape shape{a.n_slots, gridDim.x * kWaves, a.static_rounds, a.chunk_tiles};
    refill::Cursor cur = refill::make_cursor(shape, blockIdx.x * kWaves + wave);
    refill::Fresh fresh = refill::make_fresh();
    uint32_t hit_head = 0u, hit_count = 0u;
    TravStats st, sst; st.nodes = 0; st.tris = 0; sst.nodes = 0; sst.tris = 0;
    uint32_t w_paths = 0u, w_rays = 0u, w_hits0 = 0u, w_alive0 = 0u, w_rays0 = 0u, w_parked = 0u;
    bool has_ray = false;
    uint32_t slot = 0u, rng_s = 0u, depth = 0u;
    bool in_medium = false;
    V3 porg = v3s(0.0f), pdir = v3s(0.0f), thr = v3s(1.0f), lightp = v3s(0.0f);
    float pdf = 1.0f;
    for (;;) {
        asm volatile("" : "+s"(ka));
        const VPT_KERNARG WholeScene<STRICT, PLAIN>& usc = static_cast<const VPT_KERNARG WholeScene<STRICT, PLAIN>&>(ka->sc);
        const VPT_KERNARG WholeParams& uP = static_cast<const VPT_KERNARG WholeParams&>(ka->P);
        const VPT_KERNARG PathState& ups = ka->ps;
        if (hit_count >= 64u || (refill::exhausted(cur, fresh) && hit_count > 0u)) {
            const uint32_t cnt = hit_count < 64u ? hit_count : 64u;
            const bool valid = lane_id() < cnt;
            uint32_t nrays = 0u;
            bool first = false, alive = false;
            if (valid) {
                const uint32_t q = (hit_head + lane_id()) & 127u;
                ShadeIn in_;
                const float4 a = r_ra[wave][q], b = r_rb[wave][q], t = r_rt[wave][q];
                slot = r_slot[wave][q];
                in_.rng = __float_as_uint(a.w);
                in_.porg = xyz(a); in_.pdir = xyz(b);
                const uint32_t dw = __float_as_uint(b.w);
                in_.depth = dw & 0x7fffffffu; in_.in_medium = (dw >> 31) != 0u;
                in_.thr_prev = xyz(t); in_.prev_pdf = t.w;
                in_.vdepth = 0u; in_.cchan = -1; in_.vol_index = -1; in_.vol_t = 0.0f; in_.atm_comp = -1;
                in_.h = make_float4(r_t[wave][q], r_u[wave][q], r_v[wave][q], __uint_as_float(r_prim[wave][q]));
                in_.inst = r_inst[wave][q];
                first = in_.depth == 0u;
                ShadeOut o;
                shade_core<false, (int)kShadeTextured>(usc, uP, ups, slot, in_, o);
                const V3 light_prev = first ? v3s(0.0f) : xyz(ups.ACC[slot]);
                V3 E = o.emitted;
                if (o.want_sky) {
                    const bool rq = (uP.flags & VPT_FLAG_RAY_QUERIES) != 0u;
                    if (sky_visible<true, COUNT>(usc, lds_nodes, lds_tris, o.sky_o, o.sky_d, stack, sst, rq)) E = E + o.csky;
                    nrays++;
                }
                if (o.want_light) {
                    if (light_visible<true, COUNT>(usc, lds_nodes, lds_tris, o.light_o, o.light_d, o.light_gid, stack, sst)) E = E + o.clight;
                    nrays++;
                }
                auto finish = [&]() {
                    const V3 light = whole_finish(uP, ups, slot, E, in_.thr_prev, light_prev, o);
                    alive = o.alive;
                    if (alive) {
                        has_ray = true;
                        rng_s = o.rng; porg = o.new_o; pdir = o.new_d; depth = o.new_depth; in_medium = o.in_medium; thr = o.thr; pdf = o.new_pdf; lightp = light;
                    }
                };
                finish();
            }
            hit_head += cnt; hit_count -= cnt;
            w_rays += (uint32_t)__popcll(__ballot(nrays >= 1u)) + (uint32_t)__popcll(__ballot(nrays >= 2u));
            w_rays0 += (uint32_t)__popcll(__ballot(first && nrays >= 1u)) + (uint32_t)__popcll(__ballot(first && nrays >= 2u));
            w_alive0 += (uint32_t)__popcll(__ballot(first && alive));
        }
        if (!refill::exhausted(cur, fresh)) {
#pragma unroll 1
            for (;;) {
                const unsigned long long m_free = __ballot(!has_ray);
                if (m_free == 0ull) break;
                if (fresh.count == 0u) {
                    if (refill::range_empty(cur) && !refill::take_static(shape, cur)) {
                        const uint32_t take = refill::dyn_take(shape, cur);
                        uint32_t k = 0u;
                        if (lane_id() == 0u) k = atomicAdd(&ctr->extend_head, take);
                        refill::take_dynamic(shape, cur, __builtin_amdgcn_readfirstlane(k), take);
                    }
                    if (refill::exhausted(cur, fresh)) break;
                    const uint32_t g = refill::gen_count(cur);
                    const uint32_t dispatch_base = uP.dispatch_base_dev ? *uP.dispatch_base_dev : ka->dispatch_base;
                    uint32_t gslot = 0u, x = 0u, y = 0u, f = 0u;
                    const VPT_KERNARG WholeLaunch* kl = (const VPT_KERNARG WholeLaunch*)ka;
                    const cull::Packed rect{kl->cull_x, kl->cull_y};
                    const bool bounded = !COUNT && (rect.x != cull::kAxisAll || rect.y != cull::kAxisAll);
                    bool row_end = false, at_frame_end = false;
                    if (lane_id() < g) {
                        const uint32_t li = cur.w_next + lane_id();
                        if (uP.split != 1u) {
                            const uint32_t x0 = bounded ? cull::axis_first(rect.x) : 0u, y0 = bounded ? cull::axis_first(rect.y) : 0u;
                            deal::decode_split(x0, bounded ? x0 + cull::axis_span(rect.x) : uP.width - 1u, y0, bounded ? y0 + cull::axis_span(rect.y) : uP.height - 1u,
                                               uP.split, uP.width, uP.shard_pixels, uP.launch_off, dispatch_base, li, gslot, x, y, f);
                        } else if (bounded) {
                            const deal::Deal d{kl->deal.x0, kl->deal.rw, kl->deal.ys0, kl->deal.rect_px, 0u, kl->deal.last_in_frame, 0u, 0u};
                            deal::decode(d, uP.shard_pixels, uP.width, uP.shard_rank, uP.shard_count, li, gslot, x, y, f);
                            row_end = x == kl->deal.x0 + kl->deal.rw - 1u; at_frame_end = deal::frame_end(d, uP.shard_pixels, f, gslot);
                        } else { gslot = li; pixel_of_slot(uP, li, x, y, f); }
                        const uint32_t seed = pcg_hash(uP.base_seed + dispatch_base + f);
                        Rng r; r.s = y + uP.width * x + seed;
                        V3 go, gd;
                        camera_ray(cam, r, x, y, go, gd);
                        const uint32_t j = lane_id();
                        f_slot[wave][j] = gslot; f_rng[wave][j] = r.s;
                        f_ox[wave][j] = go.x; f_oy[wave][j] = go.y; f_oz[wave][j] = go.z;
                        f_dx[wave][j] = gd.x; f_dy[wave][j] = gd.y; f_dz[wave][j] = gd.z;
                    }
                    const bool first_tile = cur.w_next == 0u;
                    refill::generated(cur, fresh, g);
                    __builtin_amdgcn_fence(__ATOMIC_RELEASE, "wavefront");
                    __builtin_amdgcn_wave_barrier();
                    __builtin_amdgcn_fence(__ATOMIC_ACQUIRE, "wavefront");
                    if (bounded && uP.split == 1u) {
                        unsigned long long m_end = __ballot(row_end);
                        const unsigned long long m_last = __ballot(at_frame_end);
                        if (first_tile)
                            whole_zero_run(ups.ACC, 0u, kl->deal.head);
                        const deal::Deal dz{kl->deal.x0, kl->deal.rw, kl->deal.ys0, kl->deal.rect_px, kl->deal.gap, kl->deal.last_in_frame, kl->deal.head, kl->deal.slots};
                        while (m_end != 0ull) {
                            const uint32_t b = (uint32_t)__builtin_ctzll(m_end);
                            uint32_t first, end;
                            deal::run_after(dz, uP.shard_pixels, __builtin_amdgcn_readfirstlane(f_slot[wave][b]), ((m_last >> b) & 1ull) != 0ull, first, end);
                            m_end &= m_end - 1ull;
                            whole_zero_run(ups.ACC, first, end);
                        }
                    }
                }
                const uint32_t q = fresh.head + lanes_below(m_free);
                refill::pop(fresh, (uint32_t)__popcll(m_free));
                if (!has_ray && q < fresh.head) {
                    slot = f_slot[wave][q]; rng_s = f_rng[wave][q];
                    porg = v3(f_ox[wave][q], f_oy[wave][q], f_oz[wave][q]);
                    pdir = v3(f_dx[wave][q], f_dy[wave][q], f_dz[wave][q]);
                    depth = 0u; in_medium = false; thr = v3s(1.0f); pdf = 1.0f; lightp = v3s(0.0f);
                    has_ray = true;
                }
            }
        }
        if (__ballot(has_ray) == 0ull) {
            if (refill::exhausted(cur, fresh) && hit_count == 0u) break;
            continue;
        }
        {
            HitRec hr;
            bool hit = false;
            if (has_ray) hit = trace_any<true, COUNT>(usc, lds_nodes, lds_tris, porg, normalize(pdir), 0.01f, 100000.0f, stack, hr, st);
            const unsigned long long mh = __ballot(has_ray && hit);
            if (has_ray && hit) {
                const uint32_t q = (hit_head + hit_count + lanes_below(mh)) & 127u;
                r_slot[wave][q] = slot; r_t[wave][q] = hr.t; r_u[wave][q] = hr.u; r_v[wave][q] = hr.v; r_prim[wave][q] = hr.gid; r_inst[wave][q] = hr.inst;
                r_ra[wave][q] = f4u(porg, rng_s);
                r_rb[wave][q] = f4u(pdir, depth | (in_medium ? 0x80000000u : 0u));
                r_rt[wave][q] = f4(thr, pdf);
                if (depth != 0u) ups.ACC[slot] = f4(lightp, 0.0f);
            }
            hit_count += (uint32_t)__popcll(mh);
            w_paths += (uint32_t)__popcll(__ballot(has_ray));
            w_hits0 += (uint32_t)__popcll(__ballot(has_ray && hit && depth == 0u));
            w_parked += (uint32_t)__popcll(__ballot(has_ray && hit && depth != 0u));
            if (has_ray && !hit) {
                ShadeIn in_;
                in_.rng = rng_s; in_.porg = porg; in_.pdir = pdir; in_.depth = depth; in_.in_medium = in_medium; in_.thr_prev = thr; in_.prev_pdf = pdf;
                in_.vdepth = 0u; in_.cchan = -1; in_.vol_index = -1; in_.vol_t = 0.0f; in_.atm_comp = -1;
                in_.h = make_float4(-1.0f, 0.0f, 0.0f, 0.0f); in_.inst = 0u;
                ShadeOut o;
                shade_core<false, (int)kShadeMiss>(usc, uP, ups, slot, in_, o);
                (void)whole_finish(uP, ups, slot, o.emitted, thr, lightp, o);
            }
            has_ray = false;
            porg = v3s(0.0f); pdir = v3s(0.0f); thr = v3s(1.0f); lightp = v3s(0.0f); pdf = 1.0f; rng_s = 0u; depth = 0u; in_medium = false;
            __builtin_amdgcn_fence(__ATOMIC_RELEASE, "wavefront");
            __builtin_amdgcn_wave_barrier();
            __builtin_amdgcn_fence(__ATOMIC_ACQUIRE, "wavefront");
        }
    }
    if (lane_id() == 0) {
        if (w_paths) atomicAdd(&ctr->stat_closest, (unsigned long long)w_paths);
        if (w_rays) atomicAdd(&ctr->stat_shadow, (unsigned long long)w_rays);
        if (w_hits0) atomicAdd(&ctr->stat_primary_hits, (unsigned long long)w_hits0);
        if (w_alive0) atomicAdd(&ctr->stat_primary_alive, (unsigned long long)w_alive0);
        if (w_rays0) atomicAdd(&ctr->stat_primary_rays, (unsigned long long)w_rays0);
        if (w_parked) atomicAdd(&ctr->stat_connect, (unsigned long long)w_parked);
    }
    if (!COUNT && blockIdx.x == 0u && threadIdx.x == 0u) {
        const unsigned long long culled = ((const VPT_KERNARG WholeLaunch*)ka)->culled;
        if (culled) {
            atomicAdd(&ctr->stat_closest, culled);
#if VPT_LAB
            atomicAdd(&ctr->whole_culled, (uint32_t)culled);
#endif
        }
    }
    if (COUNT) {
        atomicAdd(&ctr->stat_nodes, (unsigned long long)st.nodes);
        atomicAdd(&ctr->stat_tris, (unsigned long long)st.tris);
        atomicAdd(&ctr->stat_shadow_nodes, (unsigned long long)sst.nodes);
        atomicAdd(&ctr->stat_shadow_tris, (unsigned long long)sst.tris);
    }
}

void launch_whole(hipStream_t s, uint32_t blocks, bool count, const DeviceScene& sc, const RenderParams& P, const PathState& ps, Counters* ctr, uint32_t n_slots,
                  uint32_t dispatch_base, bool plain, uint32_t static_rounds, uint32_t chunk_tiles, cull::Packed rect, const deal::Deal& deal, uint64_t culled) {
    const size_t lds = traverse_lds_bytes(sc, true, kWholeStackRows);
    const dim3 g(blocks), b(kTraverseBlock);
    void (*k)(WholeLaunch);
    if (plain && !count && !sc.strict_hits && sc.env_black) k = k_whole<false, false, true>;
    else if (sc.strict_hits) k = count ? k_whole<true, true, false> : k_whole<false, true, false>;
    else k = count ? k_whole<true, false, false> : k_whole<false, false, false>;
    hipLaunchKernelGGL(k, g, b, lds, s, WholeLaunch{WholeArgs{sc, P, ps, ctr, n_slots, dispatch_base, static_rounds, chunk_tiles}, rect.x, rect.y, deal, culled});
}
int whole_blocks_per_cu(const DeviceScene& sc, bool plain) {
    int nb = 0;
    const size_t lds = traverse_lds_bytes(sc, true, kWholeStackRows);
    if (plain) (void)hipOccupancyMaxActiveBlocksPerMultiprocessor(&nb, k_whole<false, false, true>, kTraverseBlock, lds);
    else (void)hipOccupancyMaxActiveBlocksPerMultiprocessor(&nb, k_whole<false, false, false>, kTraverseBlock, lds);
    return nb > 0 ? nb : 1;
}

}
```

### vulkan-path-tracer_amd/csrc/traverse.hpp

```cpp
#pragma once
#include "device_types.hpp"
#include "slab.hpp"

namespace vpt {

constexpr int kStackDepth = 14;
constexpr int kStackOverflow = 82;
constexpr int kTraverseBlock = 256;
constexpr int kWholeStackRows = 6;

struct HitRec {
    float t, u, v;
    uint32_t prim, inst, gid;
    int slot;
};

struct TravStats {
    uint32_t nodes, tris;
};

template <int ROWS>
struct TravStackT {
    static constexpr int kRows = ROWS;
    static constexpr int kOverflow = kStackDepth + kStackOverflow - ROWS;
    uint32_t* lds;
    uint32_t* glob;
    int sp;
    __device__ inline void push(uint32_t v) {
        if (sp < ROWS) lds[sp * kTraverseBlock] = v;
        else if (sp < ROWS + kOverflow) glob[sp - ROWS] = v;
        sp++;
    }
    __device__ inline uint32_t pop() {
        sp--;
        return sp < ROWS ? lds[sp * kTraverseBlock] : glob[sp - ROWS];
    }
};
using TravStack = TravStackT<kStackDepth>;
constexpr int kOverflowStride = TravStackT<kWholeStackRows>::kOverflow > kStackOverflow ? TravStackT<kWholeStackRows>::kOverflow : kStackOverflow;
static_assert(kOverflowStride >= TravStackT<kStackDepth>::kOverflow && kOverflowStride >= TravStackT<kWholeStackRows>::kOverflow && kOverflowStride >= kStackOverflow,
              "a kernel's overflow stride is longer than the region the host allocates per thread");
template <int ROWS = kStackDepth>
__device__ inline TravStackT<ROWS> make_stack(unsigned char* smem, uint32_t* overflow) {
    TravStackT<ROWS> s;
    s.lds = reinterpret_cast<uint32_t*>(smem) + threadIdx.x;
    s.glob = overflow + (size_t)(blockIdx.x * blockDim.x + threadIdx.x) * TravStackT<ROWS>::kOverflow;
    s.sp = 0;
    return s;
}

struct NodeData {
    float ox, oy, oz;
    float sx, sy, sz;
    uint32_t lox, loy, loz, hix, hiy, hiz;
    int c0, c1, c2, c3;
};
__device__ inline void unpack_node(const uint4& w0, const uint4& w1, const uint4& w2, const uint4& w3, NodeData& n) {
    n.ox = __uint_as_float(w0.x); n.oy = __uint_as_float(w0.y); n.oz = __uint_as_float(w0.z); n.sx = __uint_as_float(w0.w);
    n.lox = w1.x; n.loy = w1.y; n.loz = w1.z; n.hix = w1.w; n.hiy = w2.x; n.hiz = w2.y; n.sy = __uint_as_float(w2.z); n.sz = __uint_as_float(w2.w);
    n.c0 = (int)w3.x; n.c1 = (int)w3.y; n.c2 = (int)w3.z; n.c3 = (int)w3.w;
}

struct NodeDataWide {
    float4 nearx, neary, nearz, farx, fary, farz;
    int c0, c1, c2, c3;
};

struct GlobalSceneSrc {
    using Node = NodeData;
    const BvhNode* nodes;
    const BvhTri* tris;
    bool strict;
    __device__ inline void node(int i, NodeData& n) const {
        const uint4* p = reinterpret_cast<const uint4*>(nodes + i);
        unpack_node(p[0], p[1], p[2], p[3], n);
    }
    __device__ inline void tri(int i, float4& a, float4& b, float4& c) const {
        const float4* p = reinterpret_cast<const float4*>(tris + i);
        a = p[0]; b = p[1]; c = p[2];
    }
};
struct LdsSceneSrc {
    using Node = NodeDataWide;
    const float4* nodes;
    const float4* tris;
    bool strict;
    float reach;
    __device__ inline void tri(int i, float4& a, float4& b, float4& c) const {
        const float4* p = tris + i * 3;
        a = p[0]; b = p[1]; c = p[2];
    }
};


struct RaySlab {
    V3 o, inv;
    bool negx, negy, negz;
};
template <bool STRICT> __device__ inline RaySlab make_slab(const GlobalSceneSrc&, V3 o, V3 d) {
    RaySlab r;
    r.o = o; r.inv = safe_inverse(d);
    r.negx = r.inv.x < 0.0f; r.negy = r.inv.y < 0.0f; r.negz = r.inv.z < 0.0f;
    return r;
}
struct RaySlabWide {
    V3 o, inv, oi;
    bool fused;
    int selx, sely, selz;
};
template <bool STRICT> __device__ inline RaySlabWide make_slab(const LdsSceneSrc& src, V3 o, V3 d) {
    RaySlabWide r;
    r.o = o; r.inv = safe_inverse(d); r.oi = slab_oi(o, r.inv);
    r.selx = r.inv.x < 0.0f ? 3 : 0; r.sely = r.inv.y < 0.0f ? 4 : 1; r.selz = r.inv.z < 0.0f ? 5 : 2;
    r.fused = !STRICT && __ballot(!slab_fma_ok(o, r.oi, src.reach)) == 0ull;
    if (!r.fused) r.oi = vptfp::v3(0.0f, 0.0f, 0.0f);
    return r;
}
__device__ inline void load_node(const GlobalSceneSrc& src, const RaySlab&, int i, NodeData& n) { src.node(i, n); }
__device__ inline void load_node(const LdsSceneSrc& src, const RaySlabWide& r, int i, NodeDataWide& n) {
    const float4* p = src.nodes + i * 8;
    n.nearx = p[r.selx]; n.neary = p[r.sely]; n.nearz = p[r.selz]; n.farx = p[3 - r.selx]; n.fary = p[5 - r.sely]; n.farz = p[7 - r.selz];
    float4 c = p[6];
    n.c0 = __float_as_int(c.x); n.c1 = __float_as_int(c.y); n.c2 = __float_as_int(c.z); n.c3 = __float_as_int(c.w);
}
template <int K> __device__ inline float byte_f(uint32_t w) { return (float)((w >> (8 * K)) & 0xffu); }

__device__ inline void node_entries(const NodeData& n, const RaySlab& r, float tmin, float tlimit, float& t0, float& t1, float& t2, float& t3) {
    const float ax = n.sx * r.inv.x, ay = n.sy * r.inv.y, az = n.sz * r.inv.z;
    const float bx = (n.ox - r.o.x) * r.inv.x, by = (n.oy - r.o.y) * r.inv.y, bz = (n.oz - r.o.z) * r.inv.z;
    const uint32_t nx = r.negx ? n.hix : n.lox, fx = r.negx ? n.lox : n.hix;
    const uint32_t ny = r.negy ? n.hiy : n.loy, fy = r.negy ? n.loy : n.hiy;
    const uint32_t nz = r.negz ? n.hiz : n.loz, fz = r.negz ? n.loz : n.hiz;
#define VPT_CHILD(K, T)                                                                                                     \
    {                                                                                                                       \
        float tn = fmax_(fmax_(__builtin_fmaf(byte_f<K>(nx), ax, bx), __builtin_fmaf(byte_f<K>(ny), ay, by)),               \
                         fmax_(__builtin_fmaf(byte_f<K>(nz), az, bz), tmin));                                               \
        float tf = fmin_(fmin_(__builtin_fmaf(byte_f<K>(fx), ax, bx), __builtin_fmaf(byte_f<K>(fy), ay, by)),               \
                         fmin_(__builtin_fmaf(byte_f<K>(fz), az, bz), tlimit));                                             \
        T = (tn <= tf * 1.0000005f) ? tn : kMissT;                                                                          \
    }
    VPT_CHILD(0, t0) VPT_CHILD(1, t1) VPT_CHILD(2, t2) VPT_CHILD(3, t3)
#undef VPT_CHILD
}
typedef float vpt_f2 __attribute__((ext_vector_type(2)));
__device__ inline void node_entries_pk(const NodeData& n, const RaySlab& r, float tmin, float tlimit, float& t0, float& t1, float& t2, float& t3) {
    const float ax = n.sx * r.inv.x, ay = n.sy * r.inv.y, az = n.sz * r.inv.z;
    const float bx = (n.ox - r.o.x) * r.inv.x, by = (n.oy - r.o.y) * r.inv.y, bz = (n.oz - r.o.z) * r.inv.z;
    const uint32_t nx = r.negx ? n.hix : n.lox, fx = r.negx ? n.lox : n.hix;
    const uint32_t ny = r.negy ? n.hiy : n.loy, fy = r.negy ? n.loy : n.hiy;
    const uint32_t nz = r.negz ? n.hiz : n.loz, fz = r.negz ? n.loz : n.hiz;
    const vpt_f2 ax2 = {ax, ax}, ay2 = {ay, ay}, az2 = {az, az}, bx2 = {bx, bx}, by2 = {by, by}, bz2 = {bz, bz};
#define VPT_PAIR(W, A, B, K0, K1) __builtin_elementwise_fma((vpt_f2){byte_f<K0>(W), byte_f<K1>(W)}, A, B)
    const vpt_f2 nx01 = VPT_PAIR(nx, ax2, bx2, 0, 1), nx23 = VPT_PAIR(nx, ax2, bx2, 2, 3), ny01 = VPT_PAIR(ny, ay2, by2, 0, 1), ny23 = VPT_PAIR(ny, ay2, by2, 2, 3);
    const vpt_f2 nz01 = VPT_PAIR(nz, az2, bz2, 0, 1), nz23 = VPT_PAIR(nz, az2, bz2, 2, 3);
    const vpt_f2 fx01 = VPT_PAIR(fx, ax2, bx2, 0, 1), fx23 = VPT_PAIR(fx, ax2, bx2, 2, 3), fy01 = VPT_PAIR(fy, ay2, by2, 0, 1), fy23 = VPT_PAIR(fy, ay2, by2, 2, 3);
    const vpt_f2 fz01 = VPT_PAIR(fz, az2, bz2, 0, 1), fz23 = VPT_PAIR(fz, az2, bz2, 2, 3);
#undef VPT_PAIR
    const float tn0 = fmax_(fmax_(nx01.x, ny01.x), fmax_(nz01.x, tmin)), tn1 = fmax_(fmax_(nx01.y, ny01.y), fmax_(nz01.y, tmin));
    const float tn2 = fmax_(fmax_(nx23.x, ny23.x), fmax_(nz23.x, tmin)), tn3 = fmax_(fmax_(nx23.y, ny23.y), fmax_(nz23.y, tmin));
    const vpt_f2 tf01 = {fmin_(fmin_(fx01.x, fy01.x), fmin_(fz01.x, tlimit)), fmin_(fmin_(fx01.y, fy01.y), fmin_(fz01.y, tlimit))};
    const vpt_f2 tf23 = {fmin_(fmin_(fx23.x, fy23.x), fmin_(fz23.x, tlimit)), fmin_(fmin_(fx23.y, fy23.y), fmin_(fz23.y, tlimit))};
    const vpt_f2 slack = {1.0000005f, 1.0000005f};
    const vpt_f2 s01 = tf01 * slack, s23 = tf23 * slack;
    t0 = (tn0 <= s01.x) ? tn0 : kMissT; t1 = (tn1 <= s01.y) ? tn1 : kMissT; t2 = (tn2 <= s23.x) ? tn2 : kMissT; t3 = (tn3 <= s23.y) ? tn3 : kMissT;
}
__device__ inline void node_entries(const NodeDataWide& n, const RaySlabWide& r, float tmin, float tlimit, float& t0, float& t1, float& t2, float& t3) {
    float4 nx = n.nearx, ny = n.neary, nz = n.nearz, fx = n.farx, fy = n.fary, fz = n.farz;
    if (!r.fused) {
        nx.x -= r.o.x; nx.y -= r.o.x; nx.z -= r.o.x; nx.w -= r.o.x; fx.x -= r.o.x; fx.y -= r.o.x; fx.z -= r.o.x; fx.w -= r.o.x;
        ny.x -= r.o.y; ny.y -= r.o.y; ny.z -= r.o.y; ny.w -= r.o.y; fy.x -= r.o.y; fy.y -= r.o.y; fy.z -= r.o.y; fy.w -= r.o.y;
        nz.x -= r.o.z; nz.y -= r.o.z; nz.z -= r.o.z; nz.w -= r.o.z; fz.x -= r.o.z; fz.y -= r.o.z; fz.z -= r.o.z; fz.w -= r.o.z;
    }
#define VPT_BOX(C) box_entry_dir(nx.C, ny.C, nz.C, fx.C, fy.C, fz.C, r.oi, r.inv, tmin, tlimit)
    t0 = VPT_BOX(x); t1 = VPT_BOX(y); t2 = VPT_BOX(z); t3 = VPT_BOX(w);
#undef VPT_BOX
}
__device__ inline void cswap(float& ta, int& ca, float& tb, int& cb) {
    bool sw = tb < ta;
    float tt = sw ? tb : ta; int ct = sw ? cb : ca;
    tb = sw ? ta : tb; cb = sw ? ca : cb;
    ta = tt; ca = ct;
}

template <bool COUNT, bool STRICT, class Src, class Stack>
__device__ inline bool trace_closest_pass(const Src& src, V3 o, V3 d, float tmin, float tmax, Stack stack, HitRec& best, TravStats& st,
                                          uint32_t ex0, uint32_t ex1) {
    best.t = tmax; best.u = 0.0f; best.v = 0.0f; best.prim = 0xffffffffu; best.inst = 0xffffffffu; best.gid = 0xffffffffu; best.slot = 0;
    bool found = false;
    const auto slab = make_slab<STRICT>(src, o, d);
    stack.sp = 0;
    int cur = 0;
    while (true) {
        if (cur >= 0) {
            typename Src::Node n;
            load_node(src, slab, cur, n);
            if (COUNT) st.nodes++;
            float t0, t1, t2, t3;
            node_entries(n, slab, tmin, best.t, t0, t1, t2, t3);
            int c0 = n.c0, c1 = n.c1, c2 = n.c2, c3 = n.c3;
            cswap(t0, c0, t1, c1); cswap(t2, c2, t3, c3); cswap(t0, c0, t2, c2); cswap(t1, c1, t3, c3); cswap(t1, c1, t2, c2);
            if (t0 < kMissT) {
                if (t3 < kMissT) stack.push((uint32_t)c3);
                if (t2 < kMissT) stack.push((uint32_t)c2);
                if (t1 < kMissT) stack.push((uint32_t)c1);
                cur = c0;
                continue;
            }
        } else {
            uint32_t enc = (uint32_t)(~cur);
            int first = (int)(enc >> 3), cnt = (int)(enc & 7u) + 1;
            for (int k = 0; k < cnt; k++) {
                float4 a, b, c;
                src.tri(first + k, a, b, c);
                if (COUNT) st.tris++;
                float t, u, v;
                if (vptfp::ray_triangle(o, d, vptfp::v3(a.x, a.y, a.z), vptfp::v3(a.w, b.x, b.y), vptfp::v3(b.z, b.w, c.x),
                                        tmin, tmax, &t, &u, &v)) {
                    uint32_t gid = __float_as_uint(c.w);
                    if ((!STRICT || (gid != ex0 && gid != ex1)) && (!found || t < best.t || (t == best.t && gid < best.gid))) {
                        best.t = t; best.u = u; best.v = v;
                        best.prim = __float_as_uint(c.y); best.inst = __float_as_uint(c.z); best.gid = gid;
                        if (STRICT) best.slot = first + k;
                        found = true;
                    }
                }
            }
        }
        if (stack.sp == 0) break;
        cur = (int)stack.pop();
    }
    return found;
}

template <class Src>
__device__ inline bool slot_hit_is_local(const Src& src, int slot, V3 o, V3 d, float t) {
    float4 a, b, c;
    src.tri(slot, a, b, c);
    return vptfp::hit_is_local(o, d, vptfp::v3(a.x, a.y, a.z), vptfp::v3(a.w, b.x, b.y), vptfp::v3(b.z, b.w, c.x), t);
}
template <bool COUNT, class Src, class Stack>
__device__ inline bool trace_closest_strict(const Src& src, V3 o, V3 d, float tmin, float tmax, Stack stack, HitRec& best, TravStats& st) {
    uint32_t ex0 = 0xffffffffu, ex1 = 0xffffffffu;
    while (true) {
        if (!trace_closest_pass<COUNT, true>(src, o, d, tmin, tmax, stack, best, st, ex0, ex1)) return false;
        if (slot_hit_is_local(src, best.slot, o, d, best.t)) return true;
        ex1 = ex0; ex0 = best.gid;
    }
}
template <bool COUNT, class Src, class Stack>
__device__ inline bool trace_closest(const Src& src, V3 o, V3 d, float tmin, float tmax, Stack stack, HitRec& best, TravStats& st) {
    if (!src.strict) return trace_closest_pass<COUNT, false>(src, o, d, tmin, tmax, stack, best, st, 0xffffffffu, 0xffffffffu);
    return trace_closest_strict<COUNT>(src, o, d, tmin, tmax, stack, best, st);
}

template <bool COUNT, bool LIGHT, bool STRICT, class Src, class Stack>
__device__ inline bool trace_occluded_pass(const Src& src, V3 o, V3 d, float tmin, float tmax, float t_e, uint32_t expect, Stack stack,
                                           TravStats& st, uint32_t ex0, uint32_t ex1, int& cand_slot, float& cand_t, uint32_t& cand_gid) {
    const float tlimit = LIGHT ? t_e : tmax;
    const auto slab = make_slab<STRICT>(src, o, d);
    stack.sp = 0;
    int cur = 0;
    while (true) {
        if (cur >= 0) {
            typename Src::Node n;
            load_node(src, slab, cur, n);
            if (COUNT) st.nodes++;
            float t0, t1, t2, t3;
            node_entries(n, slab, tmin, tlimit, t0, t1, t2, t3);
            int next = 0x7fffffff;
            if (t3 < kMissT) next = n.c3;
            if (t2 < kMissT) { if (next != 0x7fffffff) stack.push((uint32_t)next); next = n.c2; }
            if (t1 < kMissT) { if (next != 0x7fffffff) stack.push((uint32_t)next); next = n.c1; }
            if (t0 < kMissT) { if (next != 0x7fffffff) stack.push((uint32_t)next); next = n.c0; }
            if (next != 0x7fffffff) { cur = next; continue; }
        } else {
            uint32_t enc = (uint32_t)(~cur);
            int first = (int)(enc >> 3), cnt = (int)(enc & 7u) + 1;
            for (int k = 0; k < cnt; k++) {
                float4 a, b, c;
                src.tri(first + k, a, b, c);
                if (COUNT) st.tris++;
                float t, u, v;
                if (vptfp::ray_triangle(o, d, vptfp::v3(a.x, a.y, a.z), vptfp::v3(a.w, b.x, b.y), vptfp::v3(b.z, b.w, c.x), tmin, tmax, &t, &u, &v)) {
                    const uint32_t gid = __float_as_uint(c.w);
                    if ((!STRICT || (gid != ex0 && gid != ex1)) && (!LIGHT || t < t_e || (t == t_e && gid < expect))) {
                        if (STRICT) { cand_slot = first + k; cand_t = t; cand_gid = gid; }
                        return true;
                    }
                }
            }
        }
        if (stack.sp == 0) break;
        cur = (int)stack.pop();
    }
    return false;
}

template <bool COUNT, bool LIGHT, class Src, class Stack>
__device__ inline bool trace_occluded_strict(const Src& src, V3 o, V3 d, float tmin, float tmax, float t_e, uint32_t expect, Stack stack,
                                                   TravStats& st) {
    int slot = 0; float t = 0.0f; uint32_t gid = 0xffffffffu;
    uint32_t ex0 = 0xffffffffu, ex1 = 0xffffffffu;
    while (true) {
        if (!trace_occluded_pass<COUNT, LIGHT, true>(src, o, d, tmin, tmax, t_e, expect, stack, st, ex0, ex1, slot, t, gid)) return false;
        if (slot_hit_is_local(src, slot, o, d, t)) return true;
        ex1 = ex0; ex0 = gid;
    }
}
template <bool COUNT, bool LIGHT, class Src, class Stack>
__device__ inline bool trace_occluded(const Src& src, V3 o, V3 d, float tmin, float tmax, float t_e, uint32_t expect, Stack stack,
                                      TravStats& st) {
    int slot = 0; float t = 0.0f; uint32_t gid = 0xffffffffu;
    if (!src.strict) return trace_occluded_pass<COUNT, LIGHT, false>(src, o, d, tmin, tmax, t_e, expect, stack, st, 0xffffffffu, 0xffffffffu, slot, t, gid);
    return trace_occluded_strict<COUNT, LIGHT>(src, o, d, tmin, tmax, t_e, expect, stack, st);
}

template <bool COUNT, class Src, class Stack>
__device__ inline bool closest_is(const Src& src, V3 o, V3 d, float tmin, float tmax, uint32_t expect, uint32_t slot, Stack stack,
                                  TravStats& st) {
    float4 a, b, c;
    src.tri((int)slot, a, b, c);
    if (COUNT) st.tris++;
    float t_e, u, v;
    if (!vptfp::ray_triangle(o, d, vptfp::v3(a.x, a.y, a.z), vptfp::v3(a.w, b.x, b.y), vptfp::v3(b.z, b.w, c.x), tmin, tmax, &t_e, &u, &v)) return false;
    if (src.strict && !vptfp::hit_is_local(o, d, vptfp::v3(a.x, a.y, a.z), vptfp::v3(a.w, b.x, b.y), vptfp::v3(b.z, b.w, c.x), t_e)) return false;
    return !trace_occluded<COUNT, true>(src, o, d, tmin, tmax, t_e, expect, stack, st);
}

template <bool LDS_SCENE>
__device__ inline void stage_scene(const DeviceScene& sc, float4* lds_nodes, float4* lds_tris) {
    if (LDS_SCENE) {
        const float4* gn = reinterpret_cast<const float4*>(sc.nodes_wide);
        const float4* gt = reinterpret_cast<const float4*>(sc.tris);
        for (uint32_t i = threadIdx.x; i < sc.node_count * 8; i += blockDim.x) lds_nodes[i] = gn[i];
        for (uint32_t i = threadIdx.x; i < sc.tri_count * 3; i += blockDim.x) lds_tris[i] = gt[i];
        __syncthreads();
    }
}
template <bool LDS_SCENE, bool COUNT, class Sc, class Stack>
__device__ inline bool trace_any(const Sc& sc, const float4* lds_nodes, const float4* lds_tris, V3 o, V3 d, float tmin,
                                 float tmax, const Stack& stack, HitRec& h, TravStats& st) {
    if constexpr (LDS_SCENE) { LdsSceneSrc src{lds_nodes, lds_tris, sc.strict_hits != 0u, kSlabFmaReach * sc.scene_extent}; return trace_closest<COUNT>(src, o, d, tmin, tmax, stack, h, st); }
    else { GlobalSceneSrc src{sc.nodes, sc.tris, sc.strict_hits != 0u}; return trace_closest<COUNT>(src, o, d, tmin, tmax, stack, h, st); }
}

template <bool LDS_SCENE, bool COUNT, class Sc, class Stack>
__device__ inline bool sky_visible(const Sc& sc, const float4* lds_nodes, const float4* lds_tris, V3 o, V3 d, const Stack& stack, TravStats& st, bool rq) {
    const float tmin = rq ? 0.0001f : 0.00001f, tmax = rq ? 1000000.0f : 1000.0f;
    if (!rq) d = normalize(d);
    if constexpr (LDS_SCENE) { LdsSceneSrc src{lds_nodes, lds_tris, sc.strict_hits != 0u, kSlabFmaReach * sc.scene_extent}; return !trace_occluded<COUNT, false>(src, o, d, tmin, tmax, 0.0f, 0u, stack, st); }
    else { GlobalSceneSrc src{sc.nodes, sc.tris, sc.strict_hits != 0u}; return !trace_occluded<COUNT, false>(src, o, d, tmin, tmax, 0.0f, 0u, stack, st); }
}
template <bool LDS_SCENE, bool COUNT, class Sc, class Stack>
__device__ inline bool light_visible(const Sc& sc, const float4* lds_nodes, const float4* lds_tris, V3 o, V3 d, uint32_t gid, const Stack& stack, TravStats& st) {
    uint32_t slot = sc.tri_slot_of_gid[gid];
    if (slot == 0xffffffffu) return false;
    if constexpr (LDS_SCENE) { LdsSceneSrc src{lds_nodes, lds_tris, sc.strict_hits != 0u, kSlabFmaReach * sc.scene_extent}; return closest_is<COUNT>(src, o, d, 0.0001f, 1000000.0f, gid, slot, stack, st); }
    else { GlobalSceneSrc src{sc.nodes, sc.tris, sc.strict_hits != 0u}; return closest_is<COUNT>(src, o, d, 0.0001f, 1000000.0f, gid, slot, stack, st); }
}

}
```

Baseline: 10460 Msamples/s.

## Tag two-child BVH nodes and take a narrow traversal path in whole kernel

While staging the scene into LDS, the change marks child indices whose BVH node holds only two valid children by setting a flag bit. During closest-hit traversal in the plain, non-strict whole kernel, a wave whose lanes all point at flagged nodes loads and tests only two boxes instead of four and sorts two entries. The goal is fewer LDS reads and fewer slab tests on the small Cornell BVH. In exchange it adds a wave ballot per node step, an extra staging pass with a sync, and a lab switch to turn the path off. Only closest-hit traversal uses the narrow path; the occlusion routines just get the new template type.

```diff
diff --git a/include/vpt_lab.h b/include/vpt_lab.h
--- a/include/vpt_lab.h
+++ b/include/vpt_lab.h
@@ -19,6 +19,7 @@
 #define VPT_LAB_WHOLE_SCHED 5u
 #define VPT_LAB_WHOLE_PARTS 6u
 #define VPT_LAB_WHOLE_CULL 7u
+#define VPT_LAB_NARROW_OFF 8u
 int vpt_lab_set(vpt_ctx* ctx, uint32_t key, uint32_t value);
 int vpt_lab_whole_culled(const vpt_ctx* ctx, uint64_t* out);
 int vpt_lab_trace(vpt_ctx* ctx, uint32_t variant, uint32_t any_hit, const uint32_t* order_host, uint32_t param, uint32_t reps,
diff --git a/vulkan-path-tracer_amd/_abi.py b/vulkan-path-tracer_amd/_abi.py
--- a/vulkan-path-tracer_amd/_abi.py
+++ b/vulkan-path-tracer_amd/_abi.py
@@ -22,7 +22,7 @@
 KERNEL_COUNT = 10
 PIPELINE_AUTO, PIPELINE_FUSED, PIPELINE_STAGED = 0, 1, 2
 PIPELINE_STAGED_R1, PIPELINE_STAGED_SORTED, PIPELINE_WHOLE = 3, 4, 5
-LAB_LANES, LAB_LANE_GRID, LAB_TAIL_GRID, LAB_WHOLE_FRAMES, LAB_WHOLE_SCHED, LAB_WHOLE_PARTS, LAB_WHOLE_CULL = 1, 2, 3, 4, 5, 6, 7
+LAB_LANES, LAB_LANE_GRID, LAB_TAIL_GRID, LAB_WHOLE_FRAMES, LAB_WHOLE_SCHED, LAB_WHOLE_PARTS, LAB_WHOLE_CULL, LAB_NARROW_OFF = 1, 2, 3, 4, 5, 6, 7, 8
 ASYNC_MAX_BOUNCES = 32
 
 
diff --git a/vulkan-path-tracer_amd/_build.py b/vulkan-path-tracer_amd/_build.py
--- a/vulkan-path-tracer_amd/_build.py
+++ b/vulkan-path-tracer_amd/_build.py
@@ -9,7 +9,7 @@
 SOURCES = ["kernels_whole.hip", "kernels_finish.hip", "kernels_bounce.hip", "kernels_aux.hip", "kernels_trace.hip", "kernels_stream.hip", "kernels_media.hip", "kernels_post.hip",
            "api_context.hip", "api_scene.hip", "api_render.hip", "api_post.hip", "api_comm.hip", "bvh_build.cpp"]
 LAB_SOURCES = ["kernels_lab_r1.hip", "api_lab.hip"]
-HEADERS = ["kernels_lut.hip", "device_types.hpp", "path_plan.hpp", "scene_prep.hpp", "grid_prep.hpp", "denoise.hpp", "temporal.hpp", "kernels.hpp", "api_ctx.hpp", "shading.hpp", "traverse.hpp", "bvh_build.hpp", "bvh_refit.hpp", "volume.hpp", "atmosphere.hpp", "wave.hpp", "shade_core.hpp", "vote.hpp", "slab.hpp", "whole_refill.hpp", "whole_args.hpp", "whole_deal.hpp", "camera.hpp", "camera_cull.hpp",
+HEADERS = ["kernels_lut.hip", "device_types.hpp", "path_plan.hpp", "scene_prep.hpp", "grid_prep.hpp", "denoise.hpp", "temporal.hpp", "kernels.hpp", "api_ctx.hpp", "shading.hpp", "traverse.hpp", "bvh_build.hpp", "bvh_refit.hpp", "volume.hpp", "atmosphere.hpp", "wave.hpp", "shade_core.hpp", "vote.hpp", "slab.hpp", "node_step.hpp", "whole_refill.hpp", "whole_args.hpp", "whole_deal.hpp", "camera.hpp", "camera_cull.hpp",
            os.path.join("..", "..", "include", "vpt.h"), os.path.join("..", "..", "include", "vpt_lab.h"), os.path.join("..", "..", "include", "vpt_fp32.h")]
 FLAGS = ["--offload-arch=gfx950", "-O3", "-std=c++17", "-fPIC", "-ffp-contract=off", "-fno-fast-math",
          "-fhip-fp32-correctly-rounded-divide-sqrt", "-Wno-unused-result", "-Wno-pass-failed"]
diff --git a/vulkan-path-tracer_amd/csrc/api_ctx.hpp b/vulkan-path-tracer_amd/csrc/api_ctx.hpp
--- a/vulkan-path-tracer_amd/csrc/api_ctx.hpp
+++ b/vulkan-path-tracer_amd/csrc/api_ctx.hpp
@@ -134,6 +134,7 @@
     uint32_t lab_whole_parts = 0;
     cull::WorldBox whole_box{};
     bool lab_whole_cull = true;
+    bool lab_narrow_off = false;
     bool depth_bounded = true;
     hipEvent_t tick_ev[kTickets] = {};
     uint64_t tick_issued = 0;
diff --git a/vulkan-path-tracer_amd/csrc/api_lab.hip b/vulkan-path-tracer_amd/csrc/api_lab.hip
--- a/vulkan-path-tracer_amd/csrc/api_lab.hip
+++ b/vulkan-path-tracer_amd/csrc/api_lab.hip
@@ -15,6 +15,7 @@
     else if (key == VPT_LAB_WHOLE_FRAMES) c->lab_whole_frames = value == 0xffffu ? 0xffffffffu : value;
     else if (key == VPT_LAB_WHOLE_PARTS && value <= plan::kMaxParts) c->lab_whole_parts = value;
     else if (key == VPT_LAB_WHOLE_CULL && value <= 1u) c->lab_whole_cull = value != 0u;
+    else if (key == VPT_LAB_NARROW_OFF && value <= 1u) c->lab_narrow_off = value != 0u;
     else return VPT_ERR_INVALID_ARGUMENT;
     c->state_gen++;
     return VPT_OK;
diff --git a/vulkan-path-tracer_amd/csrc/api_render.hip b/vulkan-path-tracer_amd/csrc/api_render.hip
--- a/vulkan-path-tracer_amd/csrc/api_render.hip
+++ b/vulkan-path-tracer_amd/csrc/api_render.hip
@@ -79,7 +79,7 @@
             const uint32_t n_waves = grid * 4u, rounds = ((n_part + 63u) / 64u) / n_waves, mode = c->lab_whole_sched >> 4;
             const uint32_t static_rounds = (mode == 0u || mode == 3u) ? std::min(rounds, 1u) : mode == 1u ? (rounds >= 2u ? rounds - 1u : 0u) : rounds / 2u;
             if (i) HIPCHK(c, hipMemsetAsync(&L.ctr->extend_head, 0, 4, s));
-            TIMED(c, s, VPT_K_PRIMARY, launch_whole(s, grid, b.count, dsc, c->P, part_state(c, L, first), L.ctr, n_part, dispatch_base + first, c->scene_plain, static_rounds, std::max(1u, c->lab_whole_sched & 15u) | (mode == 3u ? 0x100u : 0u), rect, dl, culled));
+            TIMED(c, s, VPT_K_PRIMARY, launch_whole(s, grid, b.count, dsc, c->P, part_state(c, L, first), L.ctr, n_part, dispatch_base + first, c->scene_plain, static_rounds, std::max(1u, c->lab_whole_sched & 15u) | (mode == 3u ? 0x100u : 0u) | (c->lab_narrow_off ? kWholeNarrowOff : 0u), rect, dl, culled));
             if (i + 1u < sd.parts.n) {
                 HIPCHK(c, hipEventRecord(L.ev_shade, s));
                 HIPCHK(c, hipStreamWaitEvent(L.stream2, L.ev_shade, 0));
diff --git a/vulkan-path-tracer_amd/csrc/kernels.hpp b/vulkan-path-tracer_amd/csrc/kernels.hpp
--- a/vulkan-path-tracer_amd/csrc/kernels.hpp
+++ b/vulkan-path-tracer_amd/csrc/kernels.hpp
@@ -16,6 +16,7 @@
 int bounce_blocks_per_cu(bool lds_scene, const DeviceScene& sc, bool plain = false);
 void launch_whole(hipStream_t s, uint32_t blocks, bool count, const DeviceScene& sc, const RenderParams& P, const PathState& ps, Counters* ctr, uint32_t n_slots,
                   uint32_t dispatch_base, bool plain, uint32_t static_rounds, uint32_t chunk_tiles, cull::Packed rect, const deal::Deal& deal, uint64_t culled);
+constexpr uint32_t kWholeNarrowOff = 1u << 9;
 int whole_blocks_per_cu(const DeviceScene& sc, bool plain);
 void launch_finish(hipStream_t s, uint32_t blocks, bool count, const DeviceScene& sc, const RenderParams& P, const PathState& ps, const StreamState& ss, const uint32_t* queue,
                    StreamCounters* sctr, Counters* ctr, uint32_t parity);
diff --git a/vulkan-path-tracer_amd/csrc/kernels_whole.hip b/vulkan-path-tracer_amd/csrc/kernels_whole.hip
--- a/vulkan-path-tracer_amd/csrc/kernels_whole.hip
+++ b/vulkan-path-tracer_amd/csrc/kernels_whole.hip
@@ -34,7 +34,12 @@
     __shared__ CameraBlock cam;
     if (threadIdx.x == 0u) fill_camera_block(cam, P.view_inv, P.proj_inv, P.width, P.height, P.focus_distance, P.dof_strength);
     const VPT_KERNARG WholeArgs* ka = (const VPT_KERNARG WholeArgs*)__builtin_amdgcn_kernarg_segment_ptr();
-    stage_scene<true>(sc, lds_nodes, lds_tris);
+    constexpr bool NARROW = PLAIN && !COUNT && !STRICT;
+#if VPT_LAB
+    stage_scene<true, NARROW>(sc, lds_nodes, lds_tris, (a.chunk_tiles & kWholeNarrowOff) == 0u);
+#else
+    stage_scene<true, NARROW>(sc, lds_nodes, lds_tris);
+#endif
     constexpr uint32_t kWaves = kTraverseBlock / 64u;
     __shared__ uint32_t r_slot[kWaves][128], r_prim[kWaves][128], r_inst[kWaves][128];
     __shared__ float r_t[kWaves][128], r_u[kWaves][128], r_v[kWaves][128];
@@ -84,11 +89,11 @@
                 V3 E = o.emitted;
                 if (o.want_sky) {
                     const bool rq = (uP.flags & VPT_FLAG_RAY_QUERIES) != 0u;
-                    if (sky_visible<true, COUNT>(usc, lds_nodes, lds_tris, o.sky_o, o.sky_d, stack, sst, rq)) E = E + o.csky;
+                    if (sky_visible<true, COUNT, NARROW>(usc, lds_nodes, lds_tris, o.sky_o, o.sky_d, stack, sst, rq)) E = E + o.csky;
                     nrays++;
                 }
                 if (o.want_light) {
-                    if (light_visible<true, COUNT>(usc, lds_nodes, lds_tris, o.light_o, o.light_d, o.light_gid, stack, sst)) E = E + o.clight;
+                    if (light_visible<true, COUNT, NARROW>(usc, lds_nodes, lds_tris, o.light_o, o.light_d, o.light_gid, stack, sst)) E = E + o.clight;
                     nrays++;
                 }
                 auto finish = [&]() {
@@ -184,7 +189,7 @@
         {
             HitRec hr;
             bool hit = false;
-            if (has_ray) hit = trace_any<true, COUNT>(usc, lds_nodes, lds_tris, porg, normalize(pdir), 0.01f, 100000.0f, stack, hr, st);
+            if (has_ray) hit = trace_any<true, COUNT, NARROW>(usc, lds_nodes, lds_tris, porg, normalize(pdir), 0.01f, 100000.0f, stack, hr, st);
             const unsigned long long mh = __ballot(has_ray && hit);
             if (has_ray && hit) {
                 const uint32_t q = (hit_head + hit_count + lanes_below(mh)) & 127u;
diff --git a/vulkan-path-tracer_amd/csrc/node_step.hpp b/vulkan-path-tracer_amd/csrc/node_step.hpp
--- /dev/null
+++ b/vulkan-path-tracer_amd/csrc/node_step.hpp
@@ -0,0 +1,96 @@
+#pragma once
+#include "device_types.hpp"
+#include "slab.hpp"
+
+namespace vpt {
+
+constexpr int32_t kNarrowBit = 1 << 30;
+constexpr int32_t kLdsTreeMaxNodes = 3072 / (int32_t)sizeof(BvhNodeWide);
+static_assert(kLdsTreeMaxNodes < kNarrowBit, "a node index of an LDS-resident tree would reach the narrow flag");
+
+VPT_HD bool narrow_child(const BvhNodeWide* nodes, int32_t word) {
+    if (word < 0) return false;
+    const BvhNodeWide& n = nodes[word];
+    return n.minx[0] != 1.0e30f && n.minx[1] != 1.0e30f && n.minx[2] == 1.0e30f && n.minx[3] == 1.0e30f;
+}
+
+VPT_HD void cswap(float& ta, int& ca, float& tb, int& cb) {
+    bool sw = tb < ta;
+    float tt = sw ? tb : ta; int ct = sw ? cb : ca;
+    tb = sw ? ta : tb; cb = sw ? ca : cb;
+    ta = tt; ca = ct;
+}
+
+struct RaySlabWide {
+    V3 o, inv, oi;
+    bool fused;
+    int selx, sely, selz;
+};
+struct NodeDataWide {
+    float4 nearx, neary, nearz, farx, fary, farz;
+    int c0, c1, c2, c3;
+};
+struct NodeDataNarrow {
+    float2 nearx, neary, nearz, farx, fary, farz;
+};
+
+VPT_HD const float4* node_at(const float4* nodes, uint32_t word) { return nodes + (uint32_t)(word << 3); }
+
+VPT_HD void load_node_wide(const float4* p, const RaySlabWide& r, NodeDataWide& n) {
+    n.nearx = p[r.selx]; n.neary = p[r.sely]; n.nearz = p[r.selz]; n.farx = p[3 - r.selx]; n.fary = p[5 - r.sely]; n.farz = p[7 - r.selz];
+    float4 c = p[6];
+    n.c0 = (int)vptfp::f2u(c.x); n.c1 = (int)vptfp::f2u(c.y); n.c2 = (int)vptfp::f2u(c.z); n.c3 = (int)vptfp::f2u(c.w);
+}
+#define VPT_XY(V) make_float2((V).x, (V).y)
+VPT_HD void load_node_narrow(const float4* p, const RaySlabWide& r, NodeDataNarrow& n) {
+    n.nearx = VPT_XY(p[r.selx]); n.neary = VPT_XY(p[r.sely]); n.nearz = VPT_XY(p[r.selz]);
+    n.farx = VPT_XY(p[3 - r.selx]); n.fary = VPT_XY(p[5 - r.sely]); n.farz = VPT_XY(p[7 - r.selz]);
+}
+#undef VPT_XY
+VPT_HD void narrow_children(const float4* p, int& c0, int& c1) {
+    const float4& c = p[6];
+    c0 = (int)vptfp::f2u(c.x); c1 = (int)vptfp::f2u(c.y);
+}
+
+VPT_HD void node_entries(const NodeDataWide& n, const RaySlabWide& r, float tmin, float tlimit, float& t0, float& t1, float& t2, float& t3) {
+    float4 nx = n.nearx, ny = n.neary, nz = n.nearz, fx = n.farx, fy = n.fary, fz = n.farz;
+    if (!r.fused) {
+        nx.x -= r.o.x; nx.y -= r.o.x; nx.z -= r.o.x; nx.w -= r.o.x; fx.x -= r.o.x; fx.y -= r.o.x; fx.z -= r.o.x; fx.w -= r.o.x;
+        ny.x -= r.o.y; ny.y -= r.o.y; ny.z -= r.o.y; ny.w -= r.o.y; fy.x -= r.o.y; fy.y -= r.o.y; fy.z -= r.o.y; fy.w -= r.o.y;
+        nz.x -= r.o.z; nz.y -= r.o.z; nz.z -= r.o.z; nz.w -= r.o.z; fz.x -= r.o.z; fz.y -= r.o.z; fz.z -= r.o.z; fz.w -= r.o.z;
+    }
+#define VPT_BOX(C) box_entry_dir(nx.C, ny.C, nz.C, fx.C, fy.C, fz.C, r.oi, r.inv, tmin, tlimit)
+    t0 = VPT_BOX(x); t1 = VPT_BOX(y); t2 = VPT_BOX(z); t3 = VPT_BOX(w);
+#undef VPT_BOX
+}
+VPT_HD void node_entries(const NodeDataNarrow& n, const RaySlabWide& r, float tmin, float tlimit, float& t0, float& t1) {
+    float2 nx = n.nearx, ny = n.neary, nz = n.nearz, fx = n.farx, fy = n.fary, fz = n.farz;
+    if (!r.fused) {
+        nx.x -= r.o.x; nx.y -= r.o.x; fx.x -= r.o.x; fx.y -= r.o.x;
+        ny.x -= r.o.y; ny.y -= r.o.y; fy.x -= r.o.y; fy.y -= r.o.y;
+        nz.x -= r.o.z; nz.y -= r.o.z; fz.x -= r.o.z; fz.y -= r.o.z;
+    }
+#define VPT_BOX(C) box_entry_dir(nx.C, ny.C, nz.C, fx.C, fy.C, fz.C, r.oi, r.inv, tmin, tlimit)
+    t0 = VPT_BOX(x); t1 = VPT_BOX(y);
+#undef VPT_BOX
+}
+
+constexpr int kNoChild = 0x7fffffff;
+template <class Push>
+VPT_HD int closest_order(float& t0, int c0, float& t1, int c1, float& t2, int c2, float& t3, int c3, Push&& push) {
+    cswap(t0, c0, t1, c1); cswap(t2, c2, t3, c3); cswap(t0, c0, t2, c2); cswap(t1, c1, t3, c3); cswap(t1, c1, t2, c2);
+    if (!(t0 < kMissT)) return kNoChild;
+    if (t3 < kMissT) push(c3);
+    if (t2 < kMissT) push(c2);
+    if (t1 < kMissT) push(c1);
+    return c0;
+}
+template <class Push>
+VPT_HD int closest_order(float& t0, int c0, float& t1, int c1, Push&& push) {
+    cswap(t0, c0, t1, c1);
+    if (!(t0 < kMissT)) return kNoChild;
+    if (t1 < kMissT) push(c1);
+    return c0;
+}
+
+}
diff --git a/vulkan-path-tracer_amd/csrc/traverse.hpp b/vulkan-path-tracer_amd/csrc/traverse.hpp
--- a/vulkan-path-tracer_amd/csrc/traverse.hpp
+++ b/vulkan-path-tracer_amd/csrc/traverse.hpp
@@ -1,6 +1,7 @@
 #pragma once
 #include "device_types.hpp"
 #include "slab.hpp"
+#include "node_step.hpp"
 
 namespace vpt {
 
@@ -61,10 +62,6 @@
     n.c0 = (int)w3.x; n.c1 = (int)w3.y; n.c2 = (int)w3.z; n.c3 = (int)w3.w;
 }
 
-struct NodeDataWide {
-    float4 nearx, neary, nearz, farx, fary, farz;
-    int c0, c1, c2, c3;
-};
 
 struct GlobalSceneSrc {
     using Node = NodeData;
@@ -80,8 +77,10 @@
         a = p[0]; b = p[1]; c = p[2];
     }
 };
-struct LdsSceneSrc {
+template <bool NARROW>
+struct LdsSceneSrcT {
     using Node = NodeDataWide;
+    static constexpr bool kNarrow = NARROW;
     const float4* nodes;
     const float4* tris;
     bool strict;
@@ -91,6 +90,7 @@
         a = p[0]; b = p[1]; c = p[2];
     }
 };
+using LdsSceneSrc = LdsSceneSrcT<false>;
 
 
 struct RaySlab {
@@ -103,12 +103,7 @@
     r.negx = r.inv.x < 0.0f; r.negy = r.inv.y < 0.0f; r.negz = r.inv.z < 0.0f;
     return r;
 }
-struct RaySlabWide {
-    V3 o, inv, oi;
-    bool fused;
-    int selx, sely, selz;
-};
-template <bool STRICT> __device__ inline RaySlabWide make_slab(const LdsSceneSrc& src, V3 o, V3 d) {
+template <bool STRICT, bool NARROW> __device__ inline RaySlabWide make_slab(const LdsSceneSrcT<NARROW>& src, V3 o, V3 d) {
     RaySlabWide r;
     r.o = o; r.inv = safe_inverse(d); r.oi = slab_oi(o, r.inv);
     r.selx = r.inv.x < 0.0f ? 3 : 0; r.sely = r.inv.y < 0.0f ? 4 : 1; r.selz = r.inv.z < 0.0f ? 5 : 2;
@@ -117,12 +112,8 @@
     return r;
 }
 __device__ inline void load_node(const GlobalSceneSrc& src, const RaySlab&, int i, NodeData& n) { src.node(i, n); }
-__device__ inline void load_node(const LdsSceneSrc& src, const RaySlabWide& r, int i, NodeDataWide& n) {
-    const float4* p = src.nodes + i * 8;
-    n.nearx = p[r.selx]; n.neary = p[r.sely]; n.nearz = p[r.selz]; n.farx = p[3 - r.selx]; n.fary = p[5 - r.sely]; n.farz = p[7 - r.selz];
-    float4 c = p[6];
-    n.c0 = __float_as_int(c.x); n.c1 = __float_as_int(c.y); n.c2 = __float_as_int(c.z); n.c3 = __float_as_int(c.w);
-}
+__device__ inline void load_node(const LdsSceneSrcT<false>& src, const RaySlabWide& r, int i, NodeDataWide& n) { load_node_wide(src.nodes + i * 8, r, n); }
+__device__ inline void load_node(const LdsSceneSrcT<true>& src, const RaySlabWide& r, int i, NodeDataWide& n) { load_node_wide(node_at(src.nodes, (uint32_t)i), r, n); }
 template <int K> __device__ inline float byte_f(uint32_t w) { return (float)((w >> (8 * K)) & 0xffu); }
 
 __device__ inline void node_entries(const NodeData& n, const RaySlab& r, float tmin, float tlimit, float& t0, float& t1, float& t2, float& t3) {
@@ -164,23 +155,9 @@
     const vpt_f2 s01 = tf01 * slack, s23 = tf23 * slack;
     t0 = (tn0 <= s01.x) ? tn0 : kMissT; t1 = (tn1 <= s01.y) ? tn1 : kMissT; t2 = (tn2 <= s23.x) ? tn2 : kMissT; t3 = (tn3 <= s23.y) ? tn3 : kMissT;
 }
-__device__ inline void node_entries(const NodeDataWide& n, const RaySlabWide& r, float tmin, float tlimit, float& t0, float& t1, float& t2, float& t3) {
-    float4 nx = n.nearx, ny = n.neary, nz = n.nearz, fx = n.farx, fy = n.fary, fz = n.farz;
-    if (!r.fused) {
-        nx.x -= r.o.x; nx.y -= r.o.x; nx.z -= r.o.x; nx.w -= r.o.x; fx.x -= r.o.x; fx.y -= r.o.x; fx.z -= r.o.x; fx.w -= r.o.x;
-        ny.x -= r.o.y; ny.y -= r.o.y; ny.z -= r.o.y; ny.w -= r.o.y; fy.x -= r.o.y; fy.y -= r.o.y; fy.z -= r.o.y; fy.w -= r.o.y;
-        nz.x -= r.o.z; nz.y -= r.o.z; nz.z -= r.o.z; nz.w -= r.o.z; fz.x -= r.o.z; fz.y -= r.o.z; fz.z -= r.o.z; fz.w -= r.o.z;
-    }
-#define VPT_BOX(C) box_entry_dir(nx.C, ny.C, nz.C, fx.C, fy.C, fz.C, r.oi, r.inv, tmin, tlimit)
-    t0 = VPT_BOX(x); t1 = VPT_BOX(y); t2 = VPT_BOX(z); t3 = VPT_BOX(w);
-#undef VPT_BOX
-}
-__device__ inline void cswap(float& ta, int& ca, float& tb, int& cb) {
-    bool sw = tb < ta;
-    float tt = sw ? tb : ta; int ct = sw ? cb : ca;
-    tb = sw ? ta : tb; cb = sw ? ca : cb;
-    ta = tt; ca = ct;
-}
+
+template <bool STRICT, class Src> struct TakesNarrow { static constexpr bool value = false; };
+template <bool STRICT> struct TakesNarrow<STRICT, LdsSceneSrcT<true>> { static constexpr bool value = !STRICT; };
 
 template <bool COUNT, bool STRICT, class Src, class Stack>
 __device__ inline bool trace_closest_pass(const Src& src, V3 o, V3 d, float tmin, float tmax, Stack stack, HitRec& best, TravStats& st,
@@ -192,19 +169,45 @@
     int cur = 0;
     while (true) {
         if (cur >= 0) {
-            typename Src::Node n;
-            load_node(src, slab, cur, n);
-            if (COUNT) st.nodes++;
-            float t0, t1, t2, t3;
-            node_entries(n, slab, tmin, best.t, t0, t1, t2, t3);
-            int c0 = n.c0, c1 = n.c1, c2 = n.c2, c3 = n.c3;
-            cswap(t0, c0, t1, c1); cswap(t2, c2, t3, c3); cswap(t0, c0, t2, c2); cswap(t1, c1, t3, c3); cswap(t1, c1, t2, c2);
-            if (t0 < kMissT) {
-                if (t3 < kMissT) stack.push((uint32_t)c3);
-                if (t2 < kMissT) stack.push((uint32_t)c2);
-                if (t1 < kMissT) stack.push((uint32_t)c1);
-                cur = c0;
-                continue;
+            if constexpr (!TakesNarrow<STRICT, Src>::value) {
+                typename Src::Node n;
+                load_node(src, slab, cur, n);
+                if (COUNT) st.nodes++;
+                float t0, t1, t2, t3;
+                node_entries(n, slab, tmin, best.t, t0, t1, t2, t3);
+                int c0 = n.c0, c1 = n.c1, c2 = n.c2, c3 = n.c3;
+                cswap(t0, c0, t1, c1); cswap(t2, c2, t3, c3); cswap(t0, c0, t2, c2); cswap(t1, c1, t3, c3); cswap(t1, c1, t2, c2);
+                if (t0 < kMissT) {
+                    if (t3 < kMissT) stack.push((uint32_t)c3);
+                    if (t2 < kMissT) stack.push((uint32_t)c2);
+                    if (t1 < kMissT) stack.push((uint32_t)c1);
+                    cur = c0;
+                    continue;
+                }
+            } else {
+                if (COUNT) st.nodes++;
+                const bool narrow = __ballot(cur < kNarrowBit) == 0ull;
+                const auto push = [&](int w) { stack.push((uint32_t)w); };
+                int next;
+                if (narrow) {
+                    const float4* p = node_at(src.nodes, (uint32_t)cur);
+                    float t0, t1;
+                    {
+                        NodeDataNarrow n;
+                        load_node_narrow(p, slab, n);
+                        node_entries(n, slab, tmin, best.t, t0, t1);
+                    }
+                    int c0, c1;
+                    narrow_children(p, c0, c1);
+                    next = closest_order(t0, c0, t1, c1, push);
+                } else {
+                    typename Src::Node n;
+                    load_node(src, slab, cur, n);
+                    float t0, t1, t2, t3;
+                    node_entries(n, slab, tmin, best.t, t0, t1, t2, t3);
+                    next = closest_order(t0, n.c0, t1, n.c1, t2, n.c2, t3, n.c3, push);
+                }
+                if (next != kNoChild) { cur = next; continue; }
             }
         } else {
             uint32_t enc = (uint32_t)(~cur);
@@ -327,35 +330,44 @@
     return !trace_occluded<COUNT, true>(src, o, d, tmin, tmax, t_e, expect, stack, st);
 }
 
-template <bool LDS_SCENE>
-__device__ inline void stage_scene(const DeviceScene& sc, float4* lds_nodes, float4* lds_tris) {
+template <bool LDS_SCENE, bool NARROW = false>
+__device__ inline void stage_scene(const DeviceScene& sc, float4* lds_nodes, float4* lds_tris, bool flag = true) {
     if (LDS_SCENE) {
         const float4* gn = reinterpret_cast<const float4*>(sc.nodes_wide);
         const float4* gt = reinterpret_cast<const float4*>(sc.tris);
         for (uint32_t i = threadIdx.x; i < sc.node_count * 8; i += blockDim.x) lds_nodes[i] = gn[i];
         for (uint32_t i = threadIdx.x; i < sc.tri_count * 3; i += blockDim.x) lds_tris[i] = gt[i];
         __syncthreads();
-    }
-}
-template <bool LDS_SCENE, bool COUNT, class Sc, class Stack>
+        if (NARROW) {
+            if (flag)
+                for (uint32_t i = threadIdx.x; i < sc.node_count * 4; i += blockDim.x) {
+                    int32_t* w = reinterpret_cast<int32_t*>(lds_nodes + (i >> 2) * 8 + 6) + (i & 3u);
+                    const int32_t word = *w;
+                    if (word < (int32_t)sc.node_count && narrow_child(reinterpret_cast<const BvhNodeWide*>(lds_nodes), word)) *w = word | kNarrowBit;
+                }
+            __syncthreads();
+        }
+    }
+}
+template <bool LDS_SCENE, bool COUNT, bool NARROW = false, class Sc, class Stack>
 __device__ inline bool trace_any(const Sc& sc, const float4* lds_nodes, const float4* lds_tris, V3 o, V3 d, float tmin,
                                  float tmax, const Stack& stack, HitRec& h, TravStats& st) {
-    if constexpr (LDS_SCENE) { LdsSceneSrc src{lds_nodes, lds_tris, sc.strict_hits != 0u, kSlabFmaReach * sc.scene_extent}; return trace_closest<COUNT>(src, o, d, tmin, tmax, stack, h, st); }
+    if constexpr (LDS_SCENE) { LdsSceneSrcT<NARROW> src{lds_nodes, lds_tris, sc.strict_hits != 0u, kSlabFmaReach * sc.scene_extent}; return trace_closest<COUNT>(src, o, d, tmin, tmax, stack, h, st); }
     else { GlobalSceneSrc src{sc.nodes, sc.tris, sc.strict_hits != 0u}; return trace_closest<COUNT>(src, o, d, tmin, tmax, stack, h, st); }
 }
 
-template <bool LDS_SCENE, bool COUNT, class Sc, class Stack>
+template <bool LDS_SCENE, bool COUNT, bool NARROW = false, class Sc, class Stack>
 __device__ inline bool sky_visible(const Sc& sc, const float4* lds_nodes, const float4* lds_tris, V3 o, V3 d, const Stack& stack, TravStats& st, bool rq) {
     const float tmin = rq ? 0.0001f : 0.00001f, tmax = rq ? 1000000.0f : 1000.0f;
     if (!rq) d = normalize(d);
-    if constexpr (LDS_SCENE) { LdsSceneSrc src{lds_nodes, lds_tris, sc.strict_hits != 0u, kSlabFmaReach * sc.scene_extent}; return !trace_occluded<COUNT, false>(src, o, d, tmin, tmax, 0.0f, 0u, stack, st); }
+    if constexpr (LDS_SCENE) { LdsSceneSrcT<NARROW> src{lds_nodes, lds_tris, sc.strict_hits != 0u, kSlabFmaReach * sc.scene_extent}; return !trace_occluded<COUNT, false>(src, o, d, tmin, tmax, 0.0f, 0u, stack, st); }
     else { GlobalSceneSrc src{sc.nodes, sc.tris, sc.strict_hits != 0u}; return !trace_occluded<COUNT, false>(src, o, d, tmin, tmax, 0.0f, 0u, stack, st); }
 }
-template <bool LDS_SCENE, bool COUNT, class Sc, class Stack>
+template <bool LDS_SCENE, bool COUNT, bool NARROW = false, class Sc, class Stack>
 __device__ inline bool light_visible(const Sc& sc, const float4* lds_nodes, const float4* lds_tris, V3 o, V3 d, uint32_t gid, const Stack& stack, TravStats& st) {
     uint32_t slot = sc.tri_slot_of_gid[gid];
     if (slot == 0xffffffffu) return false;
-    if constexpr (LDS_SCENE) { LdsSceneSrc src{lds_nodes, lds_tris, sc.strict_hits != 0u, kSlabFmaReach * sc.scene_extent}; return closest_is<COUNT>(src, o, d, 0.0001f, 1000000.0f, gid, slot, stack, st); }
+    if constexpr (LDS_SCENE) { LdsSceneSrcT<NARROW> src{lds_nodes, lds_tris, sc.strict_hits != 0u, kSlabFmaReach * sc.scene_extent}; return closest_is<COUNT>(src, o, d, 0.0001f, 1000000.0f, gid, slot, stack, st); }
     else { GlobalSceneSrc src{sc.nodes, sc.tris, sc.strict_hits != 0u}; return closest_is<COUNT>(src, o, d, 0.0001f, 1000000.0f, gid, slot, stack, st); }
 }
 
```

After: 10650 Msamples/s, median of 6. 1.02x the previous value.
